# yangao07/abPOA

Measured on NVIDIA H100. Metric: GCUPS (DP cells/s), global/convex 10 kbp, higher is better.
Workload: dtype int16 (packed int16x2 DPX arithmetic; int32 kernel only as overflow fallback)

## Files before the change

### abpoa_b200/csrc/poa_chain.cu

```cuda
#include <cuda_runtime.h>
#include <algorithm>
#include <atomic>
#include <chrono>
#include <mutex>
#include <thread>
#include <vector>
#include <stddef.h>
#include <stdio.h>
#include <stdlib.h>
#include <string.h>
#include <unistd.h>
#include "abpoa_gpu.h"
#include "poa_internal.h"
#include "poa_engine.h"
#include "poa_device.cuh"
#include "poa_chain.cuh"
#include "poa_chain_host.h"

#define CK(call) do { cudaError_t e_ = (call); if (e_ != cudaSuccess) \
    poa_die("libabpoa_b200/chain", "%s failed at %s:%d: %s", #call, __FILE__, __LINE__, cudaGetErrorString(e_)); } while (0)

extern "C" cudaError_t poa_launch_chain_dp_worker(int gap_mode, const int *gaps, PoaChainSlot *slots, PoaChainSync *sync, int n_groups,
                                                  const PoaChainParams *cp, int strand, int ps, const PoaParamsDev *prm, int ring_rows, int ring_cells,
                                                  cudaStream_t st);
extern "C" cudaError_t poa_launch_chain_align_p16(int gap_mode, const int *gaps, const PoaChainSlot *slots, const int32_t *idx, int n_jobs, int round,
                                                  const PoaChainParams *cp, int strand, int ps, const PoaParamsDev *prm, int ring_rows, int ring_cells,
                                                  cudaStream_t st);
extern "C" void poa_pick_ring(int gap_mode, int bits, int band_cells, size_t smem_budget, int *ring_rows, int *ring_cells);

static_assert(offsetof(PoaChainSync, q_tail) == 128 && offsetof(PoaChainSync, total) == 256 && offsetof(PoaChainSync, abort) == 384,
              "every polled / bumped word of PoaChainSync sits in its own 128-byte line");
static_assert(POA_GFA_HDR_WORDS == POA_GFA_HDR, "the device's GFA record header is the one poa_gfa_from_record reads");

template <bool PS>
__global__ void __launch_bounds__(POA_CHAIN_T) poa_chain_seed_kernel(PoaChainSlot *slots, const PoaChainParams *cp, int n) {
    if ((int)blockIdx.x >= n) return;
    chain_seed<PS>(&slots[blockIdx.x], cp);
}

template <bool PS>
__global__ void __launch_bounds__(POA_CHAIN_T) poa_chain_fuse_kernel(PoaChainSlot *slots, const int32_t *idx, const PoaChainParams *cp, int n, int round) {
    if ((int)blockIdx.x >= n) return;
    chain_fuse<PS>(&slots[idx[blockIdx.x]], cp, round);
}

__device__ __forceinline__ int sync_ld(const int32_t *p) { int v; asm volatile("ld.relaxed.gpu.global.s32 %0, [%1];" : "=r"(v) : "l"(p) : "memory"); return v; }
__device__ __forceinline__ void sync_st(int32_t *p, int v) { asm volatile("st.relaxed.gpu.global.s32 [%0], %1;" :: "l"(p), "r"(v) : "memory"); }
__device__ __forceinline__ unsigned long long sync_now_ns() { unsigned long long t; asm volatile("mov.u64 %0, %%globaltimer;" : "=l"(t)); return t; }

template <bool PS>
__global__ void __launch_bounds__(POA_CHAIN_T) poa_chain_fuse_worker_kernel(PoaChainSlot *slots, PoaChainSync *sync, const PoaChainParams *cp) {
    __shared__ int task_s;
    for (;;) {
        if (threadIdx.x < 32) {
            unsigned ticket = 0;
            if (threadIdx.x == 0) ticket = atomicAdd(&sync->q_head, 1u);
            ticket = __shfl_sync(0xffffffffu, ticket, 0);
            int g = -2; unsigned ns = 250, polls = 0;
            const unsigned long long t0 = sync_now_ns(), limit = sync->watchdog_ns;
            const int32_t *tasks = sync->tasks;
            for (;;) {
                if ((polls++ & 31u) == 0) {
                    const int tot = __shfl_sync(0xffffffffu, sync_ld(&sync->total), 0), ab = __shfl_sync(0xffffffffu, sync_ld(&sync->abort), 0);
                    if ((long long)ticket >= (long long)tot || ab) { g = -2; break; }
                    const unsigned late = __shfl_sync(0xffffffffu, (unsigned)(polls > 1 && sync_now_ns() - t0 > limit), 0);
                    if (late) { if (threadIdx.x == 0) sync_st(&sync->abort, 1); g = -2; break; }
                }
                g = __shfl_sync(0xffffffffu, sync_ld(&tasks[ticket]), 0);
                if (g >= 0) break;
                __nanosleep(ns); if (ns < 4000) ns <<= 1;
            }
            if (threadIdx.x == 0) task_s = g;
        }
        __syncthreads();
        const int g = task_s;
        __syncthreads();
        if (g < 0) return;
        __threadfence();
        PoaChainSlot *s = &slots[g];
        const unsigned long long t0 = sync_now_ns();
        chain_fuse<PS>(s, cp, 0);
        __syncthreads();
        __threadfence();
        __syncthreads();
        if (threadIdx.x == 0) { s->fuse_ns += sync_now_ns() - t0; __threadfence(); sync_st(&s->turn, 0); }
    }
}

__global__ void __launch_bounds__(POA_CHAIN_T) poa_chain_export_kernel(PoaChainSlot *slots, const PoaChainParams *cp, int n,
                                                                       int32_t *ex, const int64_t *ex_off, const int32_t *ex_cap) {
    if ((int)blockIdx.x >= n) return;
    PoaChainSlot *s = &slots[blockIdx.x];
    int32_t *o = ex + ex_off[blockIdx.x];
    const int K = cp->K, A = cp->A, nn = s->n_nodes;
    if (s->failed) { if (threadIdx.x == 0) o[0] = -1; return; }
    int32_t *ci = s->scr[0], *ca = s->scr[1];
    POA_PAR_FOR(v, nn) { ci[v] = s->in_cnt[v]; ca[v] = s->aln_cnt[v]; }
    __syncthreads();
    const int n_in = cta_excl_scan(ci, nn);
    __syncthreads();
    const int n_aln = cta_excl_scan(ca, nn);
    __syncthreads();
    int32_t *co = s->scr[2];
    POA_PAR_FOR(v, nn) co[v] = s->out_cnt[v];
    __syncthreads();
    const int n_out = cta_excl_scan(co, nn);
    __syncthreads();
    const int64_t words = 4 + 5ll * nn + 4ll * n_in + n_aln;
    if (words > ex_cap[blockIdx.x] || n_out != n_in) { if (threadIdx.x == 0) o[0] = -1; return; }
    int32_t *base = o + 4, *n_read = base + nn, *in_cnt = n_read + nn, *out_cnt = in_cnt + nn, *aln_cnt = out_cnt + nn;
    int32_t *in_id = aln_cnt + nn, *in_w = in_id + n_in, *out_id = in_w + n_in, *out_w = out_id + n_in, *aln = out_w + n_in;
    if (threadIdx.x == 0) { o[0] = nn; o[1] = n_in; o[2] = n_aln; o[3] = s->fused; }
    POA_PAR_FOR(v, nn) {
        base[v] = s->base[v]; n_read[v] = s->n_read[v]; in_cnt[v] = s->in_cnt[v]; out_cnt[v] = s->out_cnt[v]; aln_cnt[v] = s->aln_cnt[v];
        for (int e = 0; e < s->in_cnt[v]; ++e) { in_id[ci[v] + e] = s->in_id[(size_t)v * K + e]; in_w[ci[v] + e] = s->in_w[(size_t)v * K + e]; }
        for (int e = 0; e < s->out_cnt[v]; ++e) { out_id[co[v] + e] = s->out_id[(size_t)v * K + e]; out_w[co[v] + e] = s->out_w[(size_t)v * K + e]; }
        for (int a = 0; a < s->aln_cnt[v]; ++a) aln[ca[v] + a] = s->aln_id[(size_t)v * A + a];
    }
}

__global__ void __launch_bounds__(POA_CHAIN_T) poa_chain_consensus_kernel(PoaChainSlot *slots, const PoaChainParams *cp, int n,
                                                                          int32_t *out, unsigned long long *cursor, unsigned long long out_words, int64_t *rec_off) {
    if ((int)blockIdx.x >= n) return;
    PoaChainSlot *s = &slots[blockIdx.x];
    int32_t *tmp = s->scr[2];
    chain_cons_path(s, cp, tmp, s->n_cap);
    if (threadIdx.x != 0) return;
    const int len = tmp[0];
    if (len < 0) { rec_off[blockIdx.x] = -1; return; }
    const unsigned long long at = atomicAdd(cursor, (unsigned long long)(len + 1));
    if (at + (unsigned long long)(len + 1) > out_words) { rec_off[blockIdx.x] = -1; return; }
    for (int k = 0; k <= len; ++k) out[at + k] = tmp[k];
    rec_off[blockIdx.x] = (int64_t)at;
}

__global__ void __launch_bounds__(POA_CHAIN_T) poa_chain_msa_kernel(PoaChainSlot *slots, const PoaChainParams *cp, int n, int with_cons, int run_cons,
                                                                    int32_t *out, unsigned long long *cursor, unsigned long long rec_base,
                                                                    unsigned long long out_words, int64_t *rec_off) {
    if ((int)blockIdx.x >= n) return;
    __shared__ long long at_s;
    __shared__ int len_s;
    PoaChainSlot *s = &slots[blockIdx.x];
    if (run_cons && !s->failed && s->n_nodes >= 3) chain_cons_path(s, cp, s->scr[2], s->n_cap);
    if (threadIdx.x == 0) {
        const int msa_len = chain_msa_rank(s, cp);
        long long at = -1;
        if (msa_len > 0) {
            const unsigned long long words = 2 + ((unsigned long long)(s->n_reads + with_cons) * (unsigned long long)msa_len + 3) / 4;
            const unsigned long long a = rec_base + atomicAdd(cursor, words);
            if (a + words <= out_words) at = (long long)a;
        }
        at_s = at; len_s = msa_len;
        rec_off[blockIdx.x] = at;
        if (at >= 0) { out[at] = msa_len; out[at + 1] = s->n_reads + with_cons; }
    }
    __syncthreads();
    if (at_s < 0) return;
    chain_msa_rows(s, cp, len_s, with_cons, reinterpret_cast<uint8_t *>(out + at_s + 2));
}

__global__ void __launch_bounds__(POA_CHAIN_T) poa_chain_gfa_kernel(PoaChainSlot *slots, const PoaChainParams *cp, int n, int with_cons, int run_cons,
                                                                    int32_t *out, unsigned long long *cursor, unsigned long long rec_base,
                                                                    unsigned long long out_words, int64_t *rec_off) {
    if ((int)blockIdx.x >= n) return;
    __shared__ long long at_s;
    __shared__ int32_t hdr_s[POA_GFA_HDR_WORDS];
    PoaChainSlot *s = &slots[blockIdx.x];
    if (run_cons && !s->failed && s->n_nodes >= 3) chain_cons_path(s, cp, s->scr[2], s->n_cap);
    if (threadIdx.x == 0) {
        const long long words = chain_gfa_size(s, cp, with_cons, hdr_s);
        long long at = -1;
        if (words > 0) {
            const unsigned long long a = (rec_base + atomicAdd(cursor, (unsigned long long)words + 1) + 1) & ~1ull;
            if (a + (unsigned long long)words <= out_words) at = (long long)a;
        }
        at_s = at;
        rec_off[blockIdx.x] = at;
    }
    __syncthreads();
    if (at_s < 0) return;
    chain_gfa_record(s, cp, hdr_s, out + at_s);
}

__global__ void poa_chain_path_score_kernel(const int32_t *edge_w, const int32_t *node_w, int n, int32_t *out) {
    for (int i = (int)(blockIdx.x * blockDim.x + threadIdx.x); i < n; i += (int)(gridDim.x * blockDim.x)) out[i] = chain_path_score(edge_w[i], node_w[i]);
}

static inline size_t al256(size_t x) { return (x + 255) & ~(size_t)255; }

extern "C" int poa_debug_path_scores(const int32_t *edge_w, const int32_t *node_w, int n, int32_t *out) {
    if (n <= 0) return 0;
    int32_t *d = NULL;
    const size_t b = (size_t)n * 4;
    CK(cudaMalloc((void **)&d, 3 * b));
    CK(cudaMemcpy(d, edge_w, b, cudaMemcpyHostToDevice));
    CK(cudaMemcpy(d + n, node_w, b, cudaMemcpyHostToDevice));
    poa_chain_path_score_kernel<<<(n + 255) / 256 < 4096 ? (n + 255) / 256 : 4096, 256>>>(d, d + n, n, d + 2 * (size_t)n);
    CK(cudaGetLastError());
    CK(cudaMemcpy(out, d + 2 * (size_t)n, b, cudaMemcpyDeviceToHost));
    CK(cudaFree(d));
    return n;
}

int poa_chain_eligible(const abpoa_para_t *abpt) {
    const char *off = getenv("ABPOA_GPU_NO_CHAIN");
    if (off && *off == '1') return 0;
    { const char *np = getenv("ABPOA_GPU_NO_P16"); if (np && *np == '1') return 0; }
    if (abpt->align_mode != ABPOA_GLOBAL_MODE || abpt->wb < 0) return 0;
    if (abpt->gap_mode == ABPOA_LINEAR_GAP) return 0;
    const int mf = abpt->cons_algrm == ABPOA_MF && abpt->use_read_ids && !abpt->sub_aln;
    if (abpt->cons_algrm != ABPOA_HB && !mf) return 0;
    if ((abpt->use_read_ids && !abpt->out_msa && !abpt->out_gfa && !mf) || abpt->max_n_cons > 1) return 0;
    if (abpt->zdrop > 0 || abpt->rev_cigar || !abpt->ret_cigar) return 0;
    if (abpt->put_gap_on_right || abpt->put_gap_at_end) return 0;
    if (abpt->m > POA_MAX_M) return 0;
    if (!(abpt->disable_seeding && abpt->progressive_poa == 0)) return 0;
    return 1;
}

namespace {

const int ROUNDS_EXTRA = 2;
int rounds_extra(bool strand, int n_reads) { return ROUNDS_EXTRA + (strand ? n_reads - 1 : 0); }
const double STRAND_SLAB_X = 5.0;

struct GroupPlan {
    int g;
    int n_reads, qmax; int64_t bases;
    int n_cap;
    size_t reads_bytes;
    size_t static_bytes;
    double pool_units_est;
    double rec_bytes;
};

struct Cohort {
    std::vector<int> members;
    cudaStream_t st = NULL;
    cudaEvent_t ev_end = NULL;
    std::vector<cudaEvent_t> marks;
};

double now_ms() { return std::chrono::duration<double, std::milli>(std::chrono::steady_clock::now().time_since_epoch()).count(); }

struct PinnedSlot { void *p = NULL; size_t cap = 0; bool busy = false; };
std::mutex g_pin_mu; PinnedSlot g_pin[4];
void *pinned_get(int which, size_t bytes) {
    std::lock_guard<std::mutex> lk(g_pin_mu);
    PinnedSlot &ps = g_pin[which];
    if (ps.busy) { void *q = NULL; CK(cudaHostAlloc(&q, bytes ? bytes : 1, cudaHostAllocPortable)); return q; }
    if (bytes > ps.cap) {
        if (ps.p) CK(cudaFreeHost(ps.p));
        ps.cap = bytes + bytes / 4 + 4096;
        CK(cudaHostAlloc(&ps.p, ps.cap, cudaHostAllocPortable));
    }
    ps.busy = true;
    return ps.p;
}
void pinned_put(int which, void *q) {
    std::lock_guard<std::mutex> lk(g_pin_mu);
    if (q == g_pin[which].p) g_pin[which].busy = false; else CK(cudaFreeHost(q));
}

bool launches_serialised() {
    static const bool serialised = [] {
        { const char *lb = getenv("CUDA_LAUNCH_BLOCKING"); if (lb && *lb == '1') return true; }
        for (char **v = environ; v && *v; ++v)
            if (!strncmp(*v, "CUDA_INJECTION64_PATH=", 22) || !strncmp(*v, "NV_NSIGHT_INJECTION", 19) || !strncmp(*v, "NV_COMPUTE_PROFILER", 19) ||
                !strncmp(*v, "NV_SANITIZER_INJECTION", 22) || !strncmp(*v, "NV_TPS_LAUNCH_", 14)) return true;
        if (FILE *mp = fopen("/proc/self/maps", "r")) {
            char line[512]; bool hit = false;
            while (!hit && fgets(line, sizeof line, mp))
                hit = strstr(line, "InjectionTarget") || strstr(line, "cuda-injection") || strstr(line, "libsanitizer-collection") || strstr(line, "TreeLauncherTarget");
            fclose(mp);
            if (hit) return true;
        }
        return false;
    }();
    return serialised;
}

struct ChainCall {
    int dev; poa_arena *arena; abpoa_para_t *abpt; int n_workers;
    const abpoa_gpu_group_t *groups; abpoa_gpu_group_result_t *results; PoaChainStats *stats; struct PoaEmit *emit;
    bool record, verbose;
    int m, K, A;
    int P;
    bool free_run;
    int cohorts;
    bool want_msa; int with_cons;
    bool mf;
    bool want_gfa;
    int W;
    bool export_graph;
    bool strand;
    bool qv;
    bool ps;
    int sm_count;
};

ChainCall chain_call(int dev, poa_arena *arena, abpoa_para_t *abpt, int n_workers, const abpoa_gpu_group_t *groups,
                     abpoa_gpu_group_result_t *results, const std::vector<int> &todo, int flags, PoaChainStats *stats, struct PoaEmit *emit) {
    ChainCall c;
    c.dev = dev; c.arena = arena; c.abpt = abpt; c.n_workers = n_workers; c.groups = groups; c.results = results; c.stats = stats; c.emit = emit;
    c.record = (flags & ABPOA_GPU_RECORD_READS) != 0;
    c.verbose = getenv("ABPOA_GPU_PROFILE") != NULL;
    c.m = abpt->m;
    { const char *e = getenv("ABPOA_GPU_CHAIN_K"); c.K = e && *e ? atoi(e) : (c.m > 5 ? 24 : 12); }
    c.A = c.m - 1 > 1 ? c.m - 1 : 1;
    c.P = abpt->gap_mode == ABPOA_LINEAR_GAP ? 1 : (abpt->gap_mode == ABPOA_AFFINE_GAP ? 2 : 3);
    { const char *e = getenv("ABPOA_GPU_CHAIN_COHORTS"); c.cohorts = !e ? 0 : std::max(1, std::min(16, *e ? atoi(e) : 4)); }
    const bool serialised = launches_serialised();
    { const char *e = getenv("ABPOA_GPU_CHAIN_ROUNDS"); c.free_run = e && *e ? *e != '1' : !serialised; }
    { const char *e = getenv("ABPOA_GPU_CHAIN_EXPORT_GRAPH"); c.export_graph = e && *e == '1'; }
    c.want_msa = abpt->out_msa && !abpt->out_gfa;
    c.want_gfa = abpt->out_gfa && emit != NULL;
    c.with_cons = abpt->out_cons ? 1 : 0;
    c.mf = abpt->cons_algrm == ABPOA_MF;
    c.strand = abpt->amb_strand != 0;
    c.ps = abpt->inc_path_score != 0;
    c.qv = false;
    if (abpt->use_qv)
        for (int g : todo)
            for (int i = 0; groups[g].qual_weights && i < groups[g].n_seq && !c.qv; ++i) c.qv = groups[g].qual_weights[i] != NULL;
    c.W = 0;
    if (c.want_msa || c.want_gfa) for (int g : todo) c.W = std::max(c.W, (groups[g].n_seq + 63) / 64);
    c.sm_count = 132;
    if (cudaDeviceGetAttribute(&c.sm_count, cudaDevAttrMultiProcessorCount, dev) != cudaSuccess || c.sm_count < 1) c.sm_count = 132;
    return c;
}

std::vector<GroupPlan> plan_groups(const ChainCall &c, const std::vector<int> &todo, std::vector<int> &fallback) {
    std::vector<GroupPlan> plans;
    for (int g : todo) {
        const abpoa_gpu_group_t &in = c.groups[g];
        GroupPlan p; p.g = g; p.n_reads = in.n_seq; p.qmax = 0; p.bases = 0;
        bool ok = in.n_seq >= 2;
        for (int i = 0; i < in.n_seq; ++i) {
            const int l = in.seq_lens[i];
            if (l < 1) ok = false;
            if (l > p.qmax) p.qmax = l;
            p.bases += l;
            if (ok && !poa_p16_ok(c.abpt, l, 3 * l)) ok = false;
            const int *qw = c.qv && in.qual_weights ? in.qual_weights[i] : NULL;
            for (int j = 0; ok && qw && j < l; ++j) ok = qw[j] >= 0 && qw[j] <= 255;
        }
        if (c.ps && (int64_t)in.n_seq * (c.qv ? 255 : 1) > POA_PS_MAX_NODE_W) ok = false;
        if (!ok || p.qmax > (1 << 24)) { fallback.push_back(g); continue; }
        const int64_t grow = std::min<int64_t>((int64_t)((double)p.qmax * (1.0 + 0.10 * (p.n_reads - 1))) + 256,
                                               (int64_t)((double)p.qmax * (1.0 + 0.04 * (p.n_reads - 1))) + 4096);
        p.n_cap = (int)std::min<int64_t>(2 + p.bases, grow);
        PoaChainSlot probe;
        size_t own = 0; p.reads_bytes = 0;
        chain_slot_layout(&probe, p.n_cap, p.qmax, p.n_reads, c.K, c.A, c.m, c.W, c.record, [&](size_t b) { own += al256(b); return (uint8_t *)NULL; }, c.strand, c.ps);
        chain_slot_reads(&probe, p.n_reads, p.bases, [&](size_t b) { p.reads_bytes += al256(b); return (uint8_t *)NULL; }, c.qv);
        p.static_bytes = own + p.reads_bytes;
        const size_t nc = (size_t)p.n_cap;
        p.rec_bytes = c.want_msa ? (double)(nc + 1) * 4 + 8 + (double)(p.n_reads + c.with_cons) * (double)nc + 1024 : 0.0;
        if (c.want_gfa)
            p.rec_bytes = (double)(nc + 1) * 4 + 4.0 * (POA_GFA_HDR_WORDS + 4 + 4.0 * (double)nc + (double)(p.bases + p.n_reads))
                        + 8.0 * (double)nc * (double)((p.n_reads + 63) / 64) + 1024;
        const int wmax = poa_band_halfwidth(c.abpt, p.qmax);
        const double growth = c.free_run ? 0.032 : 0.045;
        const int band_slack = c.free_run ? 0 : 32;
        const double rows_final = std::min<double>(2.0 + (double)p.bases, (double)p.qmax * (1.0 + growth * (p.n_reads - 1)) + 64);
        p.pool_units_est = rows_final * (double)((2 * wmax + 1 + band_slack + 7) / 8 + 2) * c.P;
        if (c.strand) p.pool_units_est *= STRAND_SLAB_X;
        plans.push_back(p);
    }
    return plans;
}

std::vector<std::pair<size_t, size_t>> split_waves(const std::vector<GroupPlan> &plans, size_t arena_cap, std::vector<int> &fallback) {
    const double pool_margin = 1.15;
    auto fit_from = [&](size_t from, size_t limit, size_t *need_static_out, double *need_pool_out) {
        size_t end = from, need_static = 0; double need_pool = 0;
        while (end < plans.size() && end - from < limit) {
            const size_t s2 = need_static + plans[end].static_bytes + sizeof(PoaChainSlot) + 4096;
            const double p2 = need_pool + std::max(plans[end].pool_units_est * 16.0 * pool_margin, plans[end].rec_bytes);
            if (end > from && (double)s2 + p2 + (64 << 20) > (double)arena_cap) break;
            need_static = s2; need_pool = p2; ++end;
        }
        if (need_static_out) *need_static_out = need_static;
        if (need_pool_out) *need_pool_out = need_pool;
        return end;
    };
    size_t n_waves = 0;
    for (size_t q = 0; q < plans.size(); ++n_waves) q = fit_from(q, plans.size(), NULL, NULL);
    const size_t per_wave = (plans.size() + n_waves - 1) / std::max<size_t>(n_waves, 1);
    std::vector<std::pair<size_t, size_t>> waves;
    for (size_t pos = 0; pos < plans.size();) {
        size_t need_static = 0; double need_pool = 0;
        const size_t end = fit_from(pos, per_wave, &need_static, &need_pool);
        if ((double)need_static + need_pool * 0.5 + (64 << 20) > (double)arena_cap) {
            fallback.push_back(plans[pos].g); ++pos; continue;
        }
        waves.push_back({pos, end});
        pos = end;
    }
    return waves;
}

struct Wave {
    const ChainCall &c;
    const GroupPlan *plans;
    const int nw;
    std::vector<int> &fallback;

    uint8_t *d_base = NULL; size_t total = 0, doff = 0;
    PoaChainSlot *d_slots = NULL; PoaChainParams *d_cp = NULL; PoaParamsDev *d_prm = NULL;
    unsigned long long *d_cursors = NULL;
    PoaChainSync *d_sync = NULL; int32_t *d_tasks = NULL; int64_t n_tasks = 0;
    uint8_t *d_reads = NULL; size_t reads_bytes = 0;
    int32_t *d_idx = NULL; size_t idx_n = 0;
    int64_t *d_exoff = NULL, *d_msaoff = NULL, *d_gfaoff = NULL; int32_t *d_excap = NULL;
    uint8_t *d_pool = NULL; size_t pool_bytes = 0; int32_t *d_ex = NULL;
    std::vector<PoaChainSlot> hs, fin;
    uint8_t *h_reads = NULL; int32_t *h_cons = NULL, *h_ex = NULL;
    std::vector<int64_t> h_exoff; std::vector<int32_t> h_excap; int64_t ex_words = 0;
    int band_cells = 64;
    std::vector<Cohort> coh;
    cudaStream_t s0 = NULL, st_dp = NULL;
    cudaEvent_t ev_up = NULL, ev_t0 = NULL, ev_t1 = NULL;
    int ring_rows = 2, ring_cells = 64; int gaps[4];
    bool cons_kernel = false; unsigned long long rec_base = 0, cons_words = 0;
    std::vector<int64_t> recoff, msaoff, gfaoff, words, hoff2; int64_t tot_words = 0;
    std::vector<std::vector<int32_t>> rs, rn; std::vector<std::vector<uint64_t>> rh;
    std::vector<std::vector<uint8_t>> rc;
    int n_failed = 0;
    int64_t launches = 0; uint64_t h2d = 0, d2h = 0; float dev_ms = 0.f;
    double t_wave0 = 0, t_staged = 0, t_uploaded = 0, t_enqueued = 0, t_dev_done = 0, t_copied = 0;

    Wave(const ChainCall &c_, const GroupPlan *plans_, int nw_, std::vector<int> &fallback_) : c(c_), plans(plans_), nw(nw_), fallback(fallback_) {}
    Wave(const Wave &) = delete;
    Wave &operator=(const Wave &) = delete;
    ~Wave() {
        if (d_base) poa_arena_return(c.arena, d_base, total);
        if (h_reads) pinned_put(0, h_reads);
        if (h_cons) pinned_put(2, h_cons);
        if (h_ex) pinned_put(3, h_ex);
        for (Cohort &k : coh) {
            for (cudaEvent_t ev : k.marks) cudaEventDestroy(ev);
            if (k.ev_end) cudaEventDestroy(k.ev_end);
            if (k.st) cudaStreamDestroy(k.st);
        }
        if (st_dp) cudaStreamDestroy(st_dp);
        for (cudaEvent_t ev : { ev_up, ev_t0, ev_t1 }) if (ev) cudaEventDestroy(ev);
    }

    uint8_t *dtake(size_t b) { uint8_t *q = d_base + doff; doff += al256(b); return q; }

    void run() {
        if (!carve_and_stage()) {
            for (int t = 0; t < nw; ++t) fallback.push_back(plans[t].g);
            return;
        }
        if (c.free_run) run_free_running(); else run_rounds();
        collect();
        install();
        account();
    }

    bool carve_and_stage() {
        t_wave0 = now_ms();
        total = poa_arena_capacity(c.arena);
        d_base = poa_arena_borrow(c.arena, total);
        d_slots = (PoaChainSlot *)dtake((size_t)nw * sizeof(PoaChainSlot));
        d_cp = (PoaChainParams *)dtake(sizeof(PoaChainParams));
        d_prm = (PoaParamsDev *)dtake(sizeof(PoaParamsDev));
        d_cursors = (unsigned long long *)dtake((size_t)32 * sizeof(unsigned long long));
        d_sync = (PoaChainSync *)dtake(sizeof(PoaChainSync));
        for (int t = 0; t < nw; ++t) n_tasks += plans[t].n_reads - 1;
        d_tasks = (int32_t *)dtake((size_t)std::max<int64_t>(n_tasks, 1) * 4);
        for (int t = 0; t < nw; ++t) reads_bytes += plans[t].reads_bytes;
        h_reads = (uint8_t *)pinned_get(0, reads_bytes + 256);
        d_reads = dtake(reads_bytes);
        size_t roff = 0;
        auto rtake = [&](size_t b) { uint8_t *q = d_reads + roff; roff += al256(b); return q; };
        auto gtake = [&](size_t b) { return dtake(b); };
        hs.resize((size_t)nw);
        for (int t = 0; t < nw; ++t) {
            const GroupPlan &p = plans[t];
            const abpoa_gpu_group_t &in = c.groups[p.g];
            PoaChainSlot &s = hs[t]; memset(&s, 0, sizeof s);
            chain_slot_layout(&s, p.n_cap, p.qmax, p.n_reads, c.K, c.A, c.m, c.W, c.record, gtake, c.strand, c.ps);
            chain_slot_reads(&s, p.n_reads, p.bases, rtake, c.qv);
            int32_t *hoff = (int32_t *)(h_reads + ((const uint8_t *)s.read_off - d_reads)), *hw = (int32_t *)(h_reads + ((const uint8_t *)s.read_w - d_reads));
            int acc = 0;
            for (int i = 0; i < p.n_reads; ++i) {
                hoff[i] = acc; acc += in.seq_lens[i];
                hw[i] = poa_band_halfwidth(c.abpt, in.seq_lens[i]);
                const int bc = (2 * hw[i] + 1 + 104 + 7) / 8 * 8;
                if (bc > band_cells) band_cells = bc;
            }
            hoff[p.n_reads] = acc;
        }
        {
            std::atomic<int> nx(0);
            auto copy_reads = [&]() {
                for (int t; (t = nx.fetch_add(1)) < nw;) {
                    const abpoa_gpu_group_t &in = c.groups[plans[t].g];
                    uint8_t *q = h_reads + (hs[t].reads - d_reads);
                    for (int i = 0; i < in.n_seq; ++i) { memcpy(q, in.seqs[i], (size_t)in.seq_lens[i]); q += in.seq_lens[i]; }
                    if (!c.qv) continue;
                    uint8_t *w = h_reads + (hs[t].read_qw - d_reads);
                    for (int i = 0; i < in.n_seq; ++i) {
                        const int *qw = in.qual_weights ? in.qual_weights[i] : NULL;
                        if (qw) for (int j = 0; j < in.seq_lens[i]; ++j) w[j] = (uint8_t)qw[j];
                        else memset(w, 1, (size_t)in.seq_lens[i]);
                        w += in.seq_lens[i];
                    }
                }
            };
            const int nth = reads_bytes < (8u << 20) ? 1 : std::max(1, std::min(c.n_workers, 16));
            std::vector<std::thread> th;
            for (int w = 1; w < nth; ++w) th.emplace_back(copy_reads);
            copy_reads();
            for (auto &x : th) x.join();
        }
        t_staged = now_ms();
        idx_n = (size_t)n_tasks;
        for (int t = 0; t < nw; ++t) idx_n += (size_t)rounds_extra(c.strand, plans[t].n_reads);
        d_idx = (int32_t *)dtake(std::max<size_t>(idx_n, 1) * 4);
        h_exoff.resize((size_t)nw); h_excap.resize((size_t)nw);
        for (int t = 0; t < nw; ++t) {
            const GroupPlan &p = plans[t];
            const int64_t cap = 4 + 5ll * p.n_cap + 4ll * 3 * p.n_cap + (int64_t)p.n_cap * 2;
            h_exoff[t] = ex_words; h_excap[t] = (int32_t)std::min<int64_t>(cap, INT32_MAX); ex_words += (cap + 63) & ~63ll;
        }
        d_exoff = (int64_t *)dtake((size_t)nw * 8); d_excap = (int32_t *)dtake((size_t)nw * 4);
        d_msaoff = c.want_msa ? (int64_t *)dtake((size_t)nw * 8) : NULL;
        d_gfaoff = c.want_gfa ? (int64_t *)dtake((size_t)nw * 8) : NULL;
        doff = al256(doff);
        if (doff > total) poa_die("libabpoa_b200/chain", "wave layout (%zu bytes) exceeds the arena (%zu bytes)", doff, total);
        if (doff + (size_t)ex_words * 4 + (32 << 20) > total) return false;
        d_pool = d_base + doff; pool_bytes = total - doff;
        d_ex = (int32_t *)d_pool;
        return true;
    }

    void upload_and_seed(const std::vector<int32_t> &idx) {
        for (Cohort &k : coh) { CK(cudaStreamCreateWithFlags(&k.st, cudaStreamNonBlocking)); CK(cudaEventCreate(&k.ev_end)); }
        s0 = coh[0].st;
        CK(cudaEventCreateWithFlags(&ev_up, cudaEventDisableTiming)); CK(cudaEventCreate(&ev_t0)); CK(cudaEventCreate(&ev_t1));
        const abpoa_para_t *abpt = c.abpt;
        PoaChainParams hcp; memset(&hcp, 0, sizeof hcp);
        hcp.K = c.K; hcp.A = c.A; hcp.m = c.m; hcp.max_mat = abpt->max_mat; hcp.min_mis = abpt->min_mis; hcp.o1 = abpt->gap_open1; hcp.e1 = abpt->gap_ext1;
        hcp.oe1 = abpt->gap_open1 + abpt->gap_ext1; hcp.oe2 = abpt->gap_open2 + abpt->gap_ext2; hcp.record = c.record ? 1 : 0; hcp.P = c.P; hcp.W = c.W;
        hcp.cons_algrm = c.mf ? 1 : 0; hcp.amb_strand = c.strand ? 1 : 0;
        PoaParamsDev hprm; poa_fill_params(&hprm, c.abpt, 15);
        CK(cudaMemcpyAsync(d_reads, h_reads, reads_bytes, cudaMemcpyHostToDevice, s0));
        CK(cudaMemcpyAsync(d_slots, hs.data(), (size_t)nw * sizeof(PoaChainSlot), cudaMemcpyHostToDevice, s0));
        CK(cudaMemcpyAsync(d_cp, &hcp, sizeof hcp, cudaMemcpyHostToDevice, s0));
        CK(cudaMemcpyAsync(d_prm, &hprm, sizeof hprm, cudaMemcpyHostToDevice, s0));
        if (!idx.empty()) CK(cudaMemcpyAsync(d_idx, idx.data(), idx.size() * 4, cudaMemcpyHostToDevice, s0));
        CK(cudaMemcpyAsync(d_exoff, h_exoff.data(), (size_t)nw * 8, cudaMemcpyHostToDevice, s0));
        CK(cudaMemcpyAsync(d_excap, h_excap.data(), (size_t)nw * 4, cudaMemcpyHostToDevice, s0));
        CK(cudaMemsetAsync(d_cursors, 0, (size_t)32 * sizeof(unsigned long long), s0));
        h2d = reads_bytes + (uint64_t)nw * sizeof(PoaChainSlot) + sizeof hcp + sizeof hprm + idx.size() * 4 + (uint64_t)nw * 12;
        CK(cudaEventRecord(ev_t0, s0));
        if (c.ps) poa_chain_seed_kernel<true><<<nw, POA_CHAIN_T, 0, s0>>>(d_slots, d_cp, nw);
        else poa_chain_seed_kernel<false><<<nw, POA_CHAIN_T, 0, s0>>>(d_slots, d_cp, nw);
        CK(cudaGetLastError());
        CK(cudaEventRecord(ev_up, s0));
        static const size_t smem_budget = [] { const char *e = getenv("ABPOA_GPU_SMEM_KB"); return (size_t)(e && *e ? atoi(e) : 28) * 1024; }();
        poa_pick_ring(abpt->gap_mode, 16, band_cells, smem_budget, &ring_rows, &ring_cells);
        launches = 1;
        gaps[0] = abpt->gap_ext1; gaps[1] = abpt->gap_open1 + abpt->gap_ext1; gaps[2] = abpt->gap_ext2; gaps[3] = abpt->gap_open2 + abpt->gap_ext2;
        t_uploaded = now_ms();
        for (size_t k = 1; k < coh.size(); ++k) CK(cudaStreamWaitEvent(coh[k].st, ev_up, 0));
    }

    void run_free_running() {
        coh.resize(1);
        double est_tot = 0;
        for (int t = 0; t < nw; ++t) est_tot += plans[t].pool_units_est;
        static const double slab_x = [] { const char *e = getenv("ABPOA_GPU_CHAIN_SLAB_X"); return e && *e ? atof(e) : 0.0; }();
        size_t o = 0;
        for (int t = 0; t < nw; ++t) {
            size_t share = (size_t)((double)pool_bytes * plans[t].pool_units_est / est_tot) & ~(size_t)255;
            if (slab_x > 0) share = std::min(share, (size_t)(plans[t].pool_units_est * 16.0 * slab_x) & ~(size_t)255);
            hs[t].pool_base = d_pool + o; hs[t].pool_units = share / 16; hs[t].pool_cursor = NULL;
            o += share;
        }
        upload_and_seed({});
        static const double watchdog_s = [] { const char *e = getenv("ABPOA_GPU_CHAIN_WATCHDOG_S"); return e && *e ? atof(e) : 30.0; }();
        static const int fuse_per_sm = [] { const char *e = getenv("ABPOA_GPU_CHAIN_FUSE_PER_SM"); return e && *e ? std::max(1, atoi(e)) : 1; }();
        PoaChainSync hsync; memset(&hsync, 0, sizeof hsync);
        hsync.total = (int32_t)n_tasks; hsync.watchdog_ns = (unsigned long long)(watchdog_s * 1e9); hsync.tasks = d_tasks;
        CK(cudaMemcpyAsync(d_sync, &hsync, sizeof hsync, cudaMemcpyHostToDevice, s0));
        CK(cudaMemsetAsync(d_tasks, 0xff, (size_t)std::max<int64_t>(n_tasks, 1) * 4, s0));
        CK(cudaStreamCreateWithFlags(&st_dp, cudaStreamNonBlocking));
        cudaEvent_t ev_sync; CK(cudaEventCreateWithFlags(&ev_sync, cudaEventDisableTiming));
        CK(cudaEventRecord(ev_sync, s0));
        static const int fuse_cap = [] { const char *e = getenv("ABPOA_GPU_CHAIN_FUSE_WORKERS"); return e && *e ? std::max(1, atoi(e)) : (1 << 30); }();
        const int n_fuse = std::max(1, std::min(std::min(nw, c.sm_count * fuse_per_sm), fuse_cap));
        CK(cudaFuncSetAttribute(c.ps ? poa_chain_fuse_worker_kernel<true> : poa_chain_fuse_worker_kernel<false>, cudaFuncAttributePreferredSharedMemoryCarveout,
                                cudaSharedmemCarveoutMaxShared));
        static const bool dp_first = [] { const char *e = getenv("ABPOA_GPU_CHAIN_DP_FIRST"); return e && *e == '1'; }();
        CK(cudaStreamWaitEvent(st_dp, ev_sync, 0));
        if (dp_first) CK(poa_launch_chain_dp_worker(c.abpt->gap_mode, gaps, d_slots, d_sync, nw, d_cp, c.strand, c.ps, d_prm, ring_rows, ring_cells, st_dp));
        if (c.ps) poa_chain_fuse_worker_kernel<true><<<n_fuse, POA_CHAIN_T, 0, s0>>>(d_slots, d_sync, d_cp);
        else poa_chain_fuse_worker_kernel<false><<<n_fuse, POA_CHAIN_T, 0, s0>>>(d_slots, d_sync, d_cp);
        CK(cudaGetLastError());
        if (!dp_first) CK(poa_launch_chain_dp_worker(c.abpt->gap_mode, gaps, d_slots, d_sync, nw, d_cp, c.strand, c.ps, d_prm, ring_rows, ring_cells, st_dp));
        cudaEvent_t ev_dp; CK(cudaEventCreateWithFlags(&ev_dp, cudaEventDisableTiming));
        CK(cudaEventRecord(ev_dp, st_dp));
        CK(cudaStreamWaitEvent(s0, ev_dp, 0));
        CK(cudaEventDestroy(ev_sync)); CK(cudaEventDestroy(ev_dp));
        launches += 2;
    }

    void run_rounds() {
        const int n_coh = c.cohorts ? c.cohorts : std::max(1, std::min(16, (nw + c.sm_count - 1) / c.sm_count));
        coh.resize((size_t)std::min(n_coh, nw));
        for (int t = 0; t < nw; ++t) coh[(size_t)t % coh.size()].members.push_back(t);
        std::vector<double> est(coh.size(), 0.0); double est_tot = 0;
        for (size_t k = 0; k < coh.size(); ++k) { for (int t : coh[k].members) est[k] += plans[t].pool_units_est; est_tot += est[k]; }
        size_t o = 0;
        for (size_t k = 0; k < coh.size(); ++k) {
            const size_t share = k + 1 == coh.size() ? pool_bytes - o : (size_t)((double)pool_bytes * est[k] / est_tot) & ~(size_t)255;
            for (int t : coh[k].members) { hs[t].pool_base = d_pool + o; hs[t].pool_units = share / 16; hs[t].pool_cursor = d_cursors + 2 * k; }
            o += share;
        }
        std::vector<int32_t> h_idx; std::vector<std::vector<std::pair<size_t, int>>> round_of(coh.size());
        int n_rounds = 0;
        for (int t = 0; t < nw; ++t) n_rounds = std::max(n_rounds, plans[t].n_reads - 1 + rounds_extra(c.strand, plans[t].n_reads));
        for (size_t k = 0; k < coh.size(); ++k)
            for (int r = 1; r <= n_rounds; ++r) {
                const size_t at = h_idx.size(); int cnt = 0;
                for (int t : coh[k].members) if (plans[t].n_reads + rounds_extra(c.strand, plans[t].n_reads) > r) { h_idx.push_back(t); ++cnt; }
                round_of[k].push_back({at, cnt});
            }
        if (h_idx.size() != idx_n) poa_die("libabpoa_b200/chain", "round index lists (%zu entries) do not fill their region (%zu)", h_idx.size(), idx_n);
        upload_and_seed(h_idx);
        for (int r = 1; r <= n_rounds; ++r)
            for (size_t k = 0; k < coh.size(); ++k) {
                cudaStream_t st = coh[k].st;
                const std::pair<size_t, int> &ro = round_of[k][(size_t)r - 1];
                if (ro.second == 0) continue;
                cudaEvent_t e0, e1, e2; CK(cudaEventCreate(&e0)); CK(cudaEventCreate(&e1)); CK(cudaEventCreate(&e2));
                coh[k].marks.push_back(e0); coh[k].marks.push_back(e1); coh[k].marks.push_back(e2);
                CK(cudaEventRecord(e0, st));
                CK(poa_launch_chain_align_p16(c.abpt->gap_mode, gaps, d_slots, d_idx + ro.first, ro.second, r, d_cp, c.strand, c.ps, d_prm, ring_rows, ring_cells, st));
                CK(cudaEventRecord(e1, st));
                if (c.ps) poa_chain_fuse_kernel<true><<<ro.second, POA_CHAIN_T, 0, st>>>(d_slots, d_idx + ro.first, d_cp, ro.second, r);
                else poa_chain_fuse_kernel<false><<<ro.second, POA_CHAIN_T, 0, st>>>(d_slots, d_idx + ro.first, d_cp, ro.second, r);
                CK(cudaGetLastError());
                CK(cudaEventRecord(e2, st));
                launches += 2;
            }
    }

    void collect() {
        for (size_t k = 0; k < coh.size(); ++k) CK(cudaEventRecord(coh[k].ev_end, coh[k].st));
        t_enqueued = now_ms();
        for (size_t k = 1; k < coh.size(); ++k) CK(cudaStreamWaitEvent(s0, coh[k].ev_end, 0));
        CK(cudaEventRecord(ev_t1, s0));
        const bool export_graph = c.export_graph, want_msa = c.want_msa, want_gfa = c.want_gfa;
        unsigned long long *d_ccur = d_cursors;
        int64_t *d_recoff = d_exoff;
        if (c.abpt->out_gfa) cons_kernel = !export_graph && want_gfa && c.with_cons;
        else cons_kernel = !export_graph && (!want_msa || c.with_cons);
        const bool any_rec = cons_kernel || want_msa || want_gfa;
        rec_base = export_graph ? (unsigned long long)ex_words : 0;
        if (export_graph) poa_chain_export_kernel<<<nw, POA_CHAIN_T, 0, s0>>>(d_slots, d_cp, nw, d_ex, d_exoff, d_excap);
        if (any_rec) CK(cudaMemsetAsync(d_ccur, 0, sizeof(unsigned long long), s0));
        if (cons_kernel) poa_chain_consensus_kernel<<<nw, c.mf ? POA_CHAIN_T : 32, 0, s0>>>(d_slots, d_cp, nw, d_ex, d_ccur, (unsigned long long)(pool_bytes / 4), d_recoff);
        CK(cudaGetLastError());
        launches += (export_graph || cons_kernel) ? 1 : 0;
        if (want_msa) {
            poa_chain_msa_kernel<<<nw, POA_CHAIN_T, 0, s0>>>(d_slots, d_cp, nw, c.with_cons, export_graph && c.with_cons, d_ex, d_ccur, rec_base,
                                                            (unsigned long long)(pool_bytes / 4), d_msaoff);
            CK(cudaGetLastError());
            ++launches;
        }
        if (want_gfa) {
            poa_chain_gfa_kernel<<<nw, POA_CHAIN_T, 0, s0>>>(d_slots, d_cp, nw, c.with_cons, export_graph && c.with_cons, d_ex, d_ccur, rec_base,
                                                            (unsigned long long)(pool_bytes / 4), d_gfaoff);
            CK(cudaGetLastError());
            ++launches;
        }
        fin.resize((size_t)nw);
        PoaChainSlot *h_fin = (PoaChainSlot *)pinned_get(1, (size_t)nw * sizeof(PoaChainSlot));
        CK(cudaMemcpyAsync(h_fin, d_slots, (size_t)nw * sizeof(PoaChainSlot), cudaMemcpyDeviceToHost, s0));
        CK(cudaStreamSynchronize(s0));
        CK(cudaEventElapsedTime(&dev_ms, ev_t0, ev_t1));
        memcpy(fin.data(), h_fin, (size_t)nw * sizeof(PoaChainSlot));
        pinned_put(1, h_fin);
        if (c.free_run) {
            PoaChainSync hs2; CK(cudaMemcpy(&hs2, d_sync, sizeof hs2, cudaMemcpyDeviceToHost));
            if (hs2.abort) fprintf(stderr, "[libabpoa_b200/chain] watchdog: the alignment and the fuse kernel did not make progress together within ABPOA_GPU_CHAIN_WATCHDOG_S; "
                                           "unfinished groups go to the launch engine (ABPOA_GPU_CHAIN_ROUNDS=1 selects the round schedule)\n");
        }
        t_dev_done = now_ms();
        recoff.assign((size_t)nw, -1); msaoff.assign((size_t)nw, -1); gfaoff.assign((size_t)nw, -1);
        if (any_rec) {
            int64_t *h_ro = NULL; CK(cudaHostAlloc((void **)&h_ro, (size_t)nw * 24 + 8, cudaHostAllocDefault));
            if (cons_kernel) CK(cudaMemcpyAsync(h_ro, d_recoff, (size_t)nw * 8, cudaMemcpyDeviceToHost, s0));
            if (want_msa) CK(cudaMemcpyAsync(h_ro + nw, d_msaoff, (size_t)nw * 8, cudaMemcpyDeviceToHost, s0));
            if (want_gfa) CK(cudaMemcpyAsync(h_ro + 2 * nw, d_gfaoff, (size_t)nw * 8, cudaMemcpyDeviceToHost, s0));
            CK(cudaMemcpyAsync(h_ro + 3 * nw, d_ccur, 8, cudaMemcpyDeviceToHost, s0));
            CK(cudaStreamSynchronize(s0));
            if (cons_kernel) memcpy(recoff.data(), h_ro, (size_t)nw * 8);
            if (want_msa) memcpy(msaoff.data(), h_ro + nw, (size_t)nw * 8);
            if (want_gfa) memcpy(gfaoff.data(), h_ro + 2 * nw, (size_t)nw * 8);
            cons_words = (unsigned long long)h_ro[3 * nw];
            CK(cudaFreeHost(h_ro));
            if (rec_base + cons_words > pool_bytes / 4) cons_words = pool_bytes / 4 - rec_base;
            h_cons = (int32_t *)pinned_get(2, (size_t)std::max<unsigned long long>(cons_words, 1) * 4);
            if (cons_words) CK(cudaMemcpyAsync(h_cons, d_ex + rec_base, (size_t)cons_words * 4, cudaMemcpyDeviceToHost, s0));
        }
        std::vector<int32_t> hdr4((size_t)nw * 4);
        if (export_graph) {
            int32_t *h_hdr = NULL; CK(cudaHostAlloc((void **)&h_hdr, (size_t)nw * 16, cudaHostAllocDefault));
            for (int t = 0; t < nw; ++t) CK(cudaMemcpyAsync(h_hdr + 4 * t, d_ex + h_exoff[t], 16, cudaMemcpyDeviceToHost, s0));
            CK(cudaStreamSynchronize(s0));
            memcpy(hdr4.data(), h_hdr, (size_t)nw * 16);
            CK(cudaFreeHost(h_hdr));
        }
        words.assign((size_t)nw, 0); hoff2.assign((size_t)nw, 0);
        for (int t = 0; t < nw; ++t) {
            const bool rec_ok = (!cons_kernel || recoff[t] >= 0) && (!want_msa || msaoff[t] >= 0) && (!want_gfa || gfaoff[t] >= 0);
            if (!export_graph) { words[t] = (!fin[t].failed && rec_ok) ? 1 : 0; continue; }
            if (fin[t].failed || hdr4[4 * t] < 2 || !rec_ok) continue;
            words[t] = 4 + 5ll * hdr4[4 * t] + 4ll * hdr4[4 * t + 1] + hdr4[4 * t + 2];
            hoff2[t] = tot_words; tot_words += words[t];
        }
        h_ex = (int32_t *)pinned_get(3, (size_t)std::max<int64_t>(tot_words, 1) * 4);
        if (export_graph) for (int t = 0; t < nw; ++t) if (words[t]) CK(cudaMemcpyAsync(h_ex + hoff2[t], d_ex + h_exoff[t], (size_t)words[t] * 4, cudaMemcpyDeviceToHost, s0));
        rs.resize((size_t)nw); rn.resize((size_t)nw); rh.resize((size_t)nw);
        if (c.record) for (int t = 0; t < nw; ++t) {
            const int nr = plans[t].n_reads;
            rs[t].resize(nr); rn[t].resize(nr); rh[t].resize(nr);
            CK(cudaMemcpyAsync(rs[t].data(), fin[t].rec_score, (size_t)nr * 4, cudaMemcpyDeviceToHost, s0));
            CK(cudaMemcpyAsync(rn[t].data(), fin[t].rec_nops, (size_t)nr * 4, cudaMemcpyDeviceToHost, s0));
            CK(cudaMemcpyAsync(rh[t].data(), fin[t].rec_hash, (size_t)nr * 8, cudaMemcpyDeviceToHost, s0));
        }
        rc.resize((size_t)nw);
        uint64_t rc_bytes = 0;
        if (c.strand) for (int t = 0; t < nw; ++t) {
            rc[t].resize((size_t)plans[t].n_reads);
            CK(cudaMemcpyAsync(rc[t].data(), fin[t].read_rc, (size_t)plans[t].n_reads, cudaMemcpyDeviceToHost, s0));
            rc_bytes += (uint64_t)plans[t].n_reads;
        }
        CK(cudaStreamSynchronize(s0));
        d2h = (uint64_t)tot_words * 4 + (uint64_t)cons_words * 4 + (uint64_t)nw * (sizeof(PoaChainSlot) + 16) + rc_bytes;
        poa_arena_return(c.arena, d_base, total); d_base = NULL;
        t_copied = now_ms();
    }

    void install() {
        std::atomic<int> next(0), failed(0);
        std::vector<int> failed_groups; std::mutex fmu;
        const int nth = std::max(1, std::min(c.n_workers, nw));
        std::vector<std::thread> th;
        for (int w = 0; w < nth; ++w)
            th.emplace_back([&]() {
                abpoa_para_t *abpt = c.abpt;
                abpoa_t *ab = abpoa_init();
                for (;;) {
                    const int t = next.fetch_add(1);
                    if (t >= nw) break;
                    const GroupPlan &p = plans[t];
                    if (fin[t].failed || !words[t] || fin[t].fused != p.n_reads) {
                        if (c.verbose) fprintf(stderr, "[chain] group %d left the device chain after %d reads (flags 0x%x)\n", p.g, fin[t].fused, fin[t].failed);
                        std::lock_guard<std::mutex> lk(fmu); failed_groups.push_back(p.g); failed += 1; continue;
                    }
                    abpoa_gpu_group_result_t *o = &c.results[p.g];
                    memset(o, 0, sizeof *o);
                    abpoa_reset(ab, abpt, p.qmax);
                    abpoa_seq_t *abs = ab->abs;
                    abs->n_seq = p.n_reads; poa_seq_reserve(abs);
                    int n_rc_dp = 0;
                    for (int i = 0; i < p.n_reads; ++i) {
                        abs->is_rc[i] = c.strand ? rc[t][i] & 1 : 0; abs->name[i].l = 0;
                        if (c.strand) n_rc_dp += rc[t][i] >> 1 & 1;
                    }
                    if (c.export_graph) poa_graph_import(ab, abpt, h_ex + hoff2[t]);
                    else if (cons_kernel) {
                        const int32_t *rec = h_cons + recoff[t];
                        const int len = rec[0];
                        std::vector<uint8_t> cb((size_t)(len > 0 ? len : 1)); std::vector<int> cc((size_t)(len > 0 ? len : 1));
                        for (int j = 0; j < len; ++j) { cb[j] = (uint8_t)(rec[1 + j] & 0xff); cc[j] = rec[1 + j] >> 8; }
                        poa_cons_install(ab, p.n_reads, len, cb.data(), cc.data());
                    }
                    if (c.want_msa) {
                        const int32_t *rec = h_cons + (msaoff[t] - (int64_t)rec_base);
                        poa_msa_install(ab, p.n_reads, rec[1], rec[0], reinterpret_cast<const uint8_t *>(rec + 2));
                    }
                    if (c.want_gfa) poa_gfa_install(ab, h_cons + (gfaoff[t] - (int64_t)rec_base));
                    poa_finish_group_result(ab, abpt, o, c.emit, p.g);
                    if (c.want_gfa) poa_gfa_install(ab, NULL);
                    o->dp_cells = fin[t].cells; o->n_aligned = p.n_reads - 1 + n_rc_dp;
                    if (c.record) {
                        const int nr = p.n_reads;
                        o->read_best_score = (int32_t *)poa_xcalloc((size_t)nr, sizeof(int32_t));
                        o->read_n_cigar = (int32_t *)poa_xcalloc((size_t)nr, sizeof(int32_t));
                        o->read_cigar_hash = (uint64_t *)poa_xcalloc((size_t)nr, sizeof(uint64_t));
                        o->read_cigar_hash[0] = 1469598103934665603ull;
                        for (int i = 1; i < nr; ++i) { o->read_best_score[i] = rs[t][i]; o->read_n_cigar[i] = rn[t][i]; o->read_cigar_hash[i] = rh[t][i]; }
                    }
                }
                abpoa_free(ab);
            });
        for (auto &x : th) x.join();
        for (int g : failed_groups) fallback.push_back(g);
        n_failed = failed.load();
    }

    void account() {
        int64_t cells = 0, alns = 0, fwd_clk = 0, bt_clk = 0;
        for (int t = 0; t < nw; ++t) if (!fin[t].failed && words[t] && fin[t].fused == plans[t].n_reads) { cells += fin[t].cells; alns += plans[t].n_reads - 1; fwd_clk += fin[t].fwd_clk; bt_clk += fin[t].bt_clk; }
        double dp_ms = 0, fuse_ms = 0, wait_ms = 0; int64_t n_marks = 0;
        if (c.free_run) {
            int khz = 0; if (cudaDeviceGetAttribute(&khz, cudaDevAttrClockRate, c.dev) != cudaSuccess || khz <= 0) khz = 1965000;
            for (int t = 0; t < nw; ++t) {
                dp_ms += (double)(fin[t].fwd_clk + fin[t].bt_clk) / (double)khz; fuse_ms += (double)fin[t].fuse_ns * 1e-6; wait_ms += (double)fin[t].wait_ns * 1e-6;
                n_marks += fin[t].fused > 0 ? fin[t].fused - 1 : 0;
            }
        } else {
            for (Cohort &k : coh)
                for (size_t j = 0; j + 2 < k.marks.size(); j += 3) {
                    float a = 0.f, b = 0.f;
                    CK(cudaEventElapsedTime(&a, k.marks[j], k.marks[j + 1])); CK(cudaEventElapsedTime(&b, k.marks[j + 1], k.marks[j + 2]));
                    dp_ms += a; fuse_ms += b; ++n_marks;
                }
        }
        if (PoaChainStats *stats = c.stats) {
            stats->device_ms += dev_ms; stats->cells += cells; stats->alignments += alns; stats->launches += launches;
            stats->h2d_bytes += h2d; stats->d2h_bytes += d2h; stats->groups_done += nw - n_failed; stats->groups_failed += n_failed;
            stats->fwd_clk += fwd_clk; stats->bt_clk += bt_clk;
            stats->dp_ms += dp_ms; stats->fuse_ms += fuse_ms; stats->dp_launches += n_marks; stats->fuse_launches += n_marks;
            stats->wait_ms += wait_ms; stats->free_running = c.free_run ? 1 : 0;
        }
        if (!c.verbose) return;
#ifdef POA_KPROF
        {
            double pf[6] = {0, 0, 0, 0, 0, 0}; double na = 0;
            for (int t = 0; t < nw; ++t) { for (int z = 0; z < 6; ++z) pf[z] += (double)fin[t].prof[z]; na += fin[t].fused > 0 ? fin[t].fused - 1 : 0; }
            double bd[5] = {0, 0, 0, 0, 0};
            for (int t = 0; t < nw; ++t) for (int z = 0; z < 5; ++z) bd[z] += (double)fin[t].btdiag[z];
            if (na > 0) fprintf(stderr, "[chain, backtrace per alignment] %.0f steps in %.0f speculative rounds, %.0f general steps costing %.0f k-cycles, "
                                        "%.1f rows with their F planes recomputed\n", bd[0] / na, bd[1] / na, bd[2] / na, bd[3] / na, bd[4] / na);
            if (na > 0) fprintf(stderr, "[chain, k-cycles/alignment] -DPOA_KPROF phases: setup %.0f pred %.0f compute %.0f store %.0f rowmax %.0f tail+prefetch %.0f\n",
                                pf[0] / na / 1e3, pf[1] / na / 1e3, pf[2] / na / 1e3, pf[3] / na / 1e3, pf[4] / na / 1e3, pf[5] / na / 1e3);
        }
#endif
        if (c.free_run)
            fprintf(stderr, "[chain] free-running: per group on average %.1f ms inside alignments + %.1f ms inside fuse (waited %.1f ms for fuse workers incl. the fuse itself), %lld alignments\n",
                    dp_ms / nw, fuse_ms / nw, wait_ms / nw, (long long)n_marks);
        else
            fprintf(stderr, "[chain] DP kernels %.1f ms + fuse kernels %.1f ms summed over %zu concurrent cohort streams (%lld rounds)\n", dp_ms, fuse_ms, coh.size(), (long long)n_marks);
        fprintf(stderr, "[chain] wave of %d groups (%zu cohorts, K=%d): stage %.0f + upload-enqueue %.0f + launch-enqueue %.0f ms, stage+launch+device %.0f ms (device %.1f ms), export copy %.0f ms, import+consensus %.0f ms; "
                        "static %.2f GB, pool %.2f GB, export %.1f MB; %d groups handed to the launch engine\n",
                nw, coh.size(), c.K, t_staged - t_wave0, t_uploaded - t_staged, t_enqueued - t_uploaded, t_dev_done - t_wave0, dev_ms, t_copied - t_dev_done, now_ms() - t_copied,
                (double)doff / 1e9, (double)pool_bytes / 1e9, (double)tot_words * 4 / 1e6, n_failed);
    }
};

}

int poa_chain_run(int dev, poa_arena *arena, abpoa_para_t *abpt, int n_workers, const abpoa_gpu_group_t *groups,
                  abpoa_gpu_group_result_t *results, const std::vector<int> &todo, int flags, std::vector<int> &fallback, PoaChainStats *stats,
                  struct PoaEmit *emit) {
    CK(cudaSetDevice(dev));
    const ChainCall c = chain_call(dev, arena, abpt, n_workers, groups, results, todo, flags, stats, emit);
    const std::vector<GroupPlan> plans = plan_groups(c, todo, fallback);
    if (plans.empty()) return 0;
    for (const std::pair<size_t, size_t> &w : split_waves(plans, poa_arena_capacity(arena), fallback))
        Wave(c, plans.data() + w.first, (int)(w.second - w.first), fallback).run();
    return 0;
}
```

### abpoa_b200/csrc/poa_chain.cuh

```cuda
#ifndef POA_CHAIN_CUH
#define POA_CHAIN_CUH

#include <math.h>
#include <stdint.h>
#include "poa_device.cuh"

#ifdef POA_CHAIN_EMUL
#define POA_DEV static inline
#define POA_PAR_FOR(i, n) for (int i = 0; i < (n); ++i)
#define POA_CTA_SYNC() do { } while (0)
#define POA_TID0 1
#define POA_SHARED static
#define POA_ATOMIC_OR(p, v) (*(p) |= (v))
#define POA_CTZ64(x) __builtin_ctzll(x)
#define POA_CHAIN_T 256
#else
#define POA_DEV __device__ __forceinline__
#define POA_PAR_FOR(i, n) for (int i = (int)threadIdx.x; i < (n); i += (int)blockDim.x)
#define POA_CTA_SYNC() __syncthreads()
#define POA_TID0 (threadIdx.x == 0)
#define POA_SHARED __shared__
#define POA_ATOMIC_OR(p, v) atomicOr((p), (v))
#define POA_CTZ64(x) (__ffsll((long long)(x)) - 1)
#define POA_CHAIN_T 256
#endif

#define POA_CF_NODE_CAP   0x01
#define POA_CF_EDGE_CAP   0x02
#define POA_CF_ALN_CAP    0x04
#define POA_CF_ORDER      0x08
#define POA_CF_BLOB_CAP   0x10
#define POA_CF_DP_STATUS  0x20
#define POA_CF_CIGAR      0x40
#define POA_CF_POOL       0x80

#define POA_ST_SKIP       9

typedef struct PoaChainParams {
    int32_t K, A;
    int32_t m, max_mat, min_mis, o1, e1, oe1, oe2;
    int32_t record;
    int32_t P;
    int32_t W;
    int32_t cons_algrm;
    int32_t amb_strand;
} PoaChainParams;

typedef struct PoaChainSlot {
    int32_t n_nodes, n_cap, pred_cap, blob_cap;
    int32_t failed;
    int32_t n_reads, fused;
    int32_t retry;
    int32_t cur;
    int64_t cells;
    int64_t fwd_clk, bt_clk;
    uint8_t *base;
    int32_t *in_cnt, *out_cnt, *aln_cnt, *n_read;
    int32_t *in_id, *in_w, *out_id, *out_w;
    int32_t *aln_id;
    int32_t *order[2];
    int32_t *node_row;
    int32_t *rem_row;
    int32_t *scr[6];
    const uint8_t *reads; const int32_t *read_off;
    const int32_t *read_w;
    PoaJobDesc jd;
    uint8_t *pool_base; unsigned long long *pool_cursor; uint64_t pool_units;
    int32_t turn;
    int32_t rsv0;
    unsigned long long wait_ns, fuse_ns;
    int64_t prof[6];
    int64_t btdiag[5];
    int32_t *rec_score, *rec_nops; uint64_t *rec_hash;
    uint64_t *read_set;
    uint8_t *read_rc;
    uint64_t *rc_cigar;
    PoaResultDev *rc_result;
    const uint8_t *read_qw;
} PoaChainSlot;

template <class Take>
static inline void chain_slot_layout(PoaChainSlot *s, int n_cap, int qmax, int n_reads, int K, int A, int m, int W, bool record, Take take,
                                     bool strand = false, bool ps = false) {
    const size_t nc = (size_t)n_cap, scr_n = nc > (size_t)qmax + 2 ? nc : (size_t)qmax + 2;
    s->n_cap = n_cap; s->pred_cap = (int32_t)(nc * 3); s->n_reads = n_reads;
    s->blob_cap = (int32_t)(256 + (nc + 1) * 8 + (size_t)s->pred_cap * 4 + 4 + (size_t)qmax + 64);
    if (ps) s->blob_cap += (int32_t)((size_t)s->pred_cap * 4 + 4 + 16);
    s->jd.cigar_cap = (int32_t)(qmax + n_cap + 8);
    s->base = (uint8_t *)take(nc);
    s->in_cnt = (int32_t *)take(nc * 4); s->out_cnt = (int32_t *)take(nc * 4); s->aln_cnt = (int32_t *)take(nc * 4); s->n_read = (int32_t *)take(nc * 4);
    s->in_id = (int32_t *)take(nc * K * 4); s->in_w = (int32_t *)take(nc * K * 4); s->out_id = (int32_t *)take(nc * K * 4); s->out_w = (int32_t *)take(nc * K * 4);
    s->aln_id = (int32_t *)take(nc * A * 4);
    s->order[0] = (int32_t *)take(nc * 4); s->order[1] = (int32_t *)take(nc * 4); s->node_row = (int32_t *)take(nc * 4); s->rem_row = (int32_t *)take(nc * 4);
    for (int k = 0; k < 6; ++k) s->scr[k] = (int32_t *)take(scr_n * 4);
    s->jd.blob = (uint8_t *)take((size_t)s->blob_cap);
    s->jd.rowinfo = (PoaRowInfo *)take(nc * sizeof(PoaRowInfo)); s->jd.rowoff = (PoaRowOff *)take(nc * sizeof(PoaRowOff));
    s->jd.cigar = (uint64_t *)take((size_t)s->jd.cigar_cap * 8);
    s->jd.qprof = (int16_t *)take((size_t)m * ((((size_t)qmax + 1 + 7) & ~(size_t)7) + 8) * 2);
    s->jd.result = (PoaResultDev *)take(sizeof(PoaResultDev));
    s->jd.btrec = (PoaBtRec *)take(nc * sizeof(PoaBtRec));
    if (record) { s->rec_score = (int32_t *)take((size_t)n_reads * 4); s->rec_nops = (int32_t *)take((size_t)n_reads * 4); s->rec_hash = (uint64_t *)take((size_t)n_reads * 8); }
    if (W > 0) s->read_set = (uint64_t *)take(nc * W * 8);
    if (strand) {
        s->read_rc = (uint8_t *)take((size_t)n_reads);
        s->rc_cigar = (uint64_t *)take((size_t)s->jd.cigar_cap * 8);
        s->rc_result = (PoaResultDev *)take(sizeof(PoaResultDev));
    }
}

template <class Take>
static inline void chain_slot_reads(PoaChainSlot *s, int n_reads, int64_t bases, Take take, bool qv = false) {
    s->reads = (const uint8_t *)take((size_t)bases);
    s->read_off = (const int32_t *)take(((size_t)n_reads + 1) * 4);
    s->read_w = (const int32_t *)take((size_t)n_reads * 4);
    if (qv) s->read_qw = (const uint8_t *)take((size_t)bases);
}

typedef struct PoaChainSync {
    unsigned int q_head; int32_t pad0[31];
    unsigned int q_tail; int32_t pad1[31];
    int32_t total; int32_t pad2[31];
    int32_t abort; int32_t pad3[31];
    unsigned long long watchdog_ns;
    int32_t *tasks;
} PoaChainSync;

#ifdef POA_CHAIN_EMUL
POA_DEV int cta_excl_scan(int32_t *a, int n) {
    int run = 0;
    for (int i = 0; i < n; ++i) { const int v = a[i]; a[i] = run; run += v; }
    return run;
}
POA_DEV void cta_incl_maxscan(int32_t *a, int n) {
    int run = INT32_MIN;
    for (int i = 0; i < n; ++i) { if (a[i] > run) run = a[i]; a[i] = run; }
}
#else
__device__ inline int cta_excl_scan(int32_t *a, int n) {
    __shared__ int warp_sum[32];
    __shared__ int carry_s;
    const int lane = threadIdx.x & 31, wid = threadIdx.x >> 5, nw = blockDim.x >> 5;
    if (threadIdx.x == 0) carry_s = 0;
    __syncthreads();
    for (int base = 0; base < n; base += blockDim.x) {
        const int i = base + threadIdx.x;
        const int v = i < n ? a[i] : 0;
        int x = v;
#pragma unroll
        for (int d = 1; d < 32; d <<= 1) { const int t = __shfl_up_sync(0xffffffffu, x, d); if (lane >= d) x += t; }
        if (lane == 31) warp_sum[wid] = x;
        __syncthreads();
        if (wid == 0) {
            int s = lane < nw ? warp_sum[lane] : 0;
#pragma unroll
            for (int d = 1; d < 32; d <<= 1) { const int t = __shfl_up_sync(0xffffffffu, s, d); if (lane >= d) s += t; }
            warp_sum[lane] = s;
        }
        __syncthreads();
        const int carry = carry_s;
        const int before = carry + (wid > 0 ? warp_sum[wid - 1] : 0) + x - v;
        if (i < n) a[i] = before;
        __syncthreads();
        if (threadIdx.x == 0) carry_s = carry + warp_sum[nw - 1];
        __syncthreads();
    }
    return carry_s;
}
__device__ inline void cta_incl_maxscan(int32_t *a, int n) {
    __shared__ int warp_max[32];
    __shared__ int carry_m;
    const int lane = threadIdx.x & 31, wid = threadIdx.x >> 5, nw = blockDim.x >> 5;
    if (threadIdx.x == 0) carry_m = INT32_MIN;
    __syncthreads();
    for (int base = 0; base < n; base += blockDim.x) {
        const int i = base + threadIdx.x;
        int x = i < n ? a[i] : INT32_MIN;
#pragma unroll
        for (int d = 1; d < 32; d <<= 1) { const int t = __shfl_up_sync(0xffffffffu, x, d); if (lane >= d) x = max(x, t); }
        if (lane == 31) warp_max[wid] = x;
        __syncthreads();
        if (wid == 0) {
            int s = lane < nw ? warp_max[lane] : INT32_MIN;
#pragma unroll
            for (int d = 1; d < 32; d <<= 1) { const int t = __shfl_up_sync(0xffffffffu, s, d); if (lane >= d) s = max(s, t); }
            warp_max[lane] = s;
        }
        __syncthreads();
        int r = max(carry_m, x);
        if (wid > 0) r = max(r, warp_max[wid - 1]);
        if (i < n) a[i] = r;
        __syncthreads();
        if (threadIdx.x == 0) carry_m = max(carry_m, warp_max[nw - 1]);
        __syncthreads();
    }
}
#endif

POA_DEV void chain_exchange_order(int32_t *ids, int32_t *ws, int n) {
    for (int j = 0; j + 1 < n; ++j)
        for (int k = j + 1; k < n; ++k)
            if (ws[j] < ws[k]) { int32_t t = ids[j]; ids[j] = ids[k]; ids[k] = t; t = ws[j]; ws[j] = ws[k]; ws[k] = t; }
}

POA_DEV int chain_group_last_row(const PoaChainSlot *s, int A, const int32_t *order, int old_n, int v) {
    int r = s->node_row[v];
    const int na = s->aln_cnt[v];
    if (na == 0) return r;
    const int32_t *al = s->aln_id + (size_t)v * A;
    for (; r + 1 < old_n; ++r) {
        const int u = order[r + 1];
        int member = 0;
        for (int a = 0; a < na; ++a) if (al[a] == u) { member = 1; break; }
        if (!member) break;
    }
    return r;
}

POA_DEV int chain_ref_pn(const PoaChainParams *cp, int qlen, int n_rows) {
    const int len = qlen > n_rows ? qlen : n_rows;
    const int a = qlen * cp->max_mat, b = len * cp->e1 + cp->o1;
    const int max_score = a > b ? a : b;
    return max_score <= 32767 - cp->min_mis - cp->oe1 - cp->oe2 ? 16 : 8;
}

POA_DEV size_t chain_al16(size_t x) { return (x + 15) & ~(size_t)15; }

POA_DEV bool chain_weak_hit(int best_score, int qlen, int node_n, int max_mat) {
    const int lim = qlen < node_n - 2 ? qlen : node_n - 2;
    return best_score < lim * max_mat * .3333;
}

#define POA_PS_MAX_NODE_W (1 << 20)
POA_DEV int chain_path_score(int edge_w, int node_w) {
    if (node_w == 0 || edge_w == 0) return 0;
    const int s = (int)round(log((double)edge_w / (double)node_w));
    return s > -20 ? s : -20;
}

POA_DEV uint8_t chain_comp(uint8_t b) { return b < 4 ? (uint8_t)(3 - b) : (uint8_t)4; }

typedef struct ChainRead { const uint8_t *q, *w; int len; bool rc; } ChainRead;

POA_DEV ChainRead chain_read(const PoaChainSlot *s, int r) {
    ChainRead rd;
    rd.q = s->reads + s->read_off[r]; rd.w = s->read_qw ? s->read_qw + s->read_off[r] : NULL;
    rd.len = s->read_off[r + 1] - s->read_off[r]; rd.rc = s->read_rc && (s->read_rc[r] & 1);
    return rd;
}

POA_DEV uint8_t chain_read_base(const ChainRead &rd, int qi) { return rd.rc ? chain_comp(rd.q[rd.len - 1 - qi]) : rd.q[qi]; }

POA_DEV int chain_read_weight(const ChainRead &rd, int qi) { return !rd.w ? 1 : rd.w[rd.rc ? rd.len - 1 - qi : qi]; }

POA_DEV void chain_set_remain(PoaChainSlot *s, int K, const int32_t *order, int n) {
    POA_SHARED int t_ptr[POA_CHAIN_T], t_val[POA_CHAIN_T], t_np[POA_CHAIN_T], t_nv[POA_CHAIN_T];
    int32_t *rem = s->rem_row;
    if (POA_TID0) rem[n - 1] = -1;
    POA_CTA_SYNC();
    for (int hi = n - 1; hi > 0; hi -= POA_CHAIN_T) {
        const int lo = hi - POA_CHAIN_T > 0 ? hi - POA_CHAIN_T : 0;
        const int cnt = hi - lo;
        POA_PAR_FOR(l, POA_CHAIN_T) {
            if (l < cnt) {
                const int v = order[lo + l];
                const int sr = s->node_row[s->out_id[(size_t)v * K]];
                if (sr >= hi) { t_ptr[l] = -1; t_val[l] = rem[sr] + 1; }
                else { t_ptr[l] = sr - lo; t_val[l] = 1; }
            } else { t_ptr[l] = -1; t_val[l] = 0; }
        }
        POA_CTA_SYNC();
        for (int step = 1; step < POA_CHAIN_T; step <<= 1) {
            POA_PAR_FOR(l, POA_CHAIN_T) {
                const int p = t_ptr[l];
                if (p >= 0) { t_nv[l] = t_val[l] + t_val[p]; t_np[l] = t_ptr[p]; } else { t_nv[l] = t_val[l]; t_np[l] = -1; }
            }
            POA_CTA_SYNC();
            POA_PAR_FOR(l, POA_CHAIN_T) { t_val[l] = t_nv[l]; t_ptr[l] = t_np[l]; }
            POA_CTA_SYNC();
        }
        POA_PAR_FOR(l, POA_CHAIN_T) { if (l < cnt) rem[lo + l] = t_val[l]; }
        POA_CTA_SYNC();
    }
}

template <bool PS = false>
POA_DEV void chain_flatten(PoaChainSlot *s, const PoaChainParams *cp, const int32_t *order, int n, int r, int pool_parity, int generous) {
    const int K = cp->K;
    int32_t *cnt = s->scr[0];
    POA_PAR_FOR(i, n) cnt[i] = i == 0 ? 0 : s->in_cnt[order[i]];
    POA_CTA_SYNC();
    const int n_pred = cta_excl_scan(cnt, n);
    POA_CTA_SYNC();
    const int qlen = s->read_off[r + 1] - s->read_off[r];
    uint8_t *blob = const_cast<uint8_t *>(s->jd.blob);
    PoaJobHeader *h = reinterpret_cast<PoaJobHeader *>(blob);
    size_t off = chain_al16(sizeof(PoaJobHeader));
    const size_t off_rowmeta = off; off += chain_al16(((size_t)n + 1) * 8);
    const size_t off_pred = off; off += chain_al16((size_t)n_pred * 4 + 4);
    const size_t off_ps = off; if (PS) off += chain_al16((size_t)n_pred * 4 + 4);
    const size_t off_qs = off; off += chain_al16((size_t)qlen + 1) + 16;
    if (off > (size_t)s->blob_cap || n_pred > s->pred_cap) {
        if (POA_TID0) { POA_ATOMIC_OR(&s->failed, POA_CF_BLOB_CAP); h->n_rows = 0; }
        POA_CTA_SYNC();
        return;
    }
    int32_t *rowmeta = reinterpret_cast<int32_t *>(blob + off_rowmeta), *pred = reinterpret_cast<int32_t *>(blob + off_pred);
    int32_t *pscore = reinterpret_cast<int32_t *>(blob + off_ps);
    uint8_t *qs = blob + off_qs;
    POA_PAR_FOR(i, n) {
        const int v = order[i];
        const int po = cnt[i];
        rowmeta[2 * i] = po;
        rowmeta[2 * i + 1] = (int32_t)((uint32_t)s->rem_row[i] << 8) | s->base[v];
        if (i > 0) {
            const int ni = s->in_cnt[v];
            const int32_t *iid = s->in_id + (size_t)v * K;
            for (int e = 0; e < ni; ++e) {
                const int pr = s->node_row[iid[e]];
                if (pr >= i) POA_ATOMIC_OR(&s->failed, POA_CF_ORDER);
                pred[po + e] = pr;
                if (PS) {
                    const int u = iid[e], no = s->out_cnt[u];
                    const int32_t *ow = s->out_w + (size_t)u * K;
                    int node_w = 0;
                    for (int o = 0; o < no; ++o) node_w += ow[o];
                    pscore[po + e] = chain_path_score(s->in_w[(size_t)v * K + e], node_w);
                }
            }
        }
    }
    const uint8_t *q = s->reads + s->read_off[r];
    const int qpad = (int)(off - off_qs);
    POA_PAR_FOR(j, qpad) qs[j] = (j >= 1 && j <= qlen) ? q[j - 1] : (uint8_t)0;
    if (POA_TID0) {
        rowmeta[2 * n] = n_pred; rowmeta[2 * n + 1] = 0;
        h->qlen = qlen; h->w = s->read_w[r]; h->node_n = n;
        h->off_rowmeta = (int32_t)off_rowmeta; h->off_pred = (int32_t)off_pred; h->off_predscore = PS ? (int32_t)off_ps : -1; h->off_live = -1;
        h->off_qs = (int32_t)off_qs; h->rsv[0] = h->rsv[1] = h->rsv[2] = h->rsv[3] = 0;
        h->blob_bytes = (int32_t)off; h->pn = chain_ref_pn(cp, qlen, n); h->pad[0] = h->pad[1] = 0;
#ifndef POA_CHAIN_EMUL
        if (s->pool_base) {
            const int w = s->read_w[r];
            const int drift = qlen > s->rem_row[0] ? qlen - s->rem_row[0] : s->rem_row[0] - qlen;
            unsigned long long per_row = (unsigned long long)((2 * w + 1 + drift + 64 + 7) / 8 + 2);
            const unsigned long long full = (unsigned long long)((qlen + 1 + 7) / 8 + 1);
            if (generous || per_row > full) per_row = full;
            const unsigned long long units = per_row * (unsigned long long)cp->P * (unsigned long long)n;
            if (!s->pool_cursor) {
                s->jd.planes = s->pool_base; s->jd.plane_cap_units = s->pool_units;
            } else {
                const unsigned long long at = atomicAdd(&s->pool_cursor[pool_parity & 1], units);
                if (at + units > s->pool_units) POA_ATOMIC_OR(&s->failed, POA_CF_POOL);
                else { s->jd.planes = s->pool_base + (size_t)at * (POA_GROUP * 2); s->jd.plane_cap_units = units; }
            }
        }
#endif
    }
    POA_CTA_SYNC();
    if (POA_TID0) h->n_rows = s->failed ? 0 : n;
    POA_CTA_SYNC();
}

template <bool PS = false>
POA_DEV void chain_seed(PoaChainSlot *s, const PoaChainParams *cp) {
    const int K = cp->K;
    ChainRead rd = chain_read(s, 0);
    rd.rc = false;
    const int len = rd.len;
    const uint8_t *q = rd.q;
    const int n = len + 2;
    if (n > s->n_cap || len < 1) {
        if (POA_TID0) { POA_ATOMIC_OR(&s->failed, POA_CF_NODE_CAP); reinterpret_cast<PoaJobHeader *>(const_cast<uint8_t *>(s->jd.blob))->n_rows = 0; }
        POA_CTA_SYNC();
        return;
    }
    int32_t *order = s->order[0];
    POA_PAR_FOR(v, n) {
        s->aln_cnt[v] = 0;
        if (v == 0) { s->base[v] = 0; s->in_cnt[v] = 0; s->out_cnt[v] = 1; s->out_id[0] = 2; s->out_w[0] = chain_read_weight(rd, 0); s->n_read[v] = 1; order[0] = 0; s->node_row[0] = 0; }
        else if (v == 1) {
            s->base[v] = 0; s->out_cnt[v] = 0; s->in_cnt[v] = 1; s->in_id[(size_t)K] = len + 1; s->in_w[(size_t)K] = chain_read_weight(rd, len - 1); s->n_read[v] = 0;
            order[n - 1] = 1; s->node_row[1] = n - 1;
        } else {
            const int i = v - 2;
            s->base[v] = q[i];
            s->in_cnt[v] = 1; s->in_id[(size_t)v * K] = i == 0 ? 0 : v - 1; s->in_w[(size_t)v * K] = chain_read_weight(rd, i);
            s->out_cnt[v] = 1; s->out_id[(size_t)v * K] = i == len - 1 ? 1 : v + 1; s->out_w[(size_t)v * K] = chain_read_weight(rd, i == len - 1 ? i : i + 1);
            s->n_read[v] = 1;
            order[i + 1] = v; s->node_row[v] = i + 1;
        }
    }
    if (cp->W > 0) {
        const int W = cp->W;
        POA_PAR_FOR(v, n) { uint64_t *rs = s->read_set + (size_t)v * W; for (int wd = 0; wd < W; ++wd) rs[wd] = (wd == 0 && v != 1) ? 1ull : 0ull; }
    }
    if (POA_TID0) { s->n_nodes = n; s->cur = 0; s->fused = 1; s->retry = 0; if (s->read_rc) s->read_rc[0] = 0; }
    POA_CTA_SYNC();
    chain_set_remain(s, K, order, n);
    if (s->n_reads > 1) chain_flatten<PS>(s, cp, order, n, 1, 1, 0);
}

#define CK_OLD  0
#define CK_NEWM 1
#define CK_NEWI 2

template <bool PS = false>
POA_DEV void chain_fuse(PoaChainSlot *s, const PoaChainParams *cp, int round) {
    const int K = cp->K, A = cp->A;
    const int r = s->fused;
    PoaJobHeader *hdr = reinterpret_cast<PoaJobHeader *>(const_cast<uint8_t *>(s->jd.blob));
    if (s->failed || r >= s->n_reads) return;
    const PoaResultDev *res = s->jd.result;
    if (res->status == POA_ST_SKIP) return;
    if (res->status == POA_ST_PLANE_OVF && !s->retry && s->pool_cursor) {
        POA_CTA_SYNC();
        if (POA_TID0) s->retry = 1;
        chain_flatten<PS>(s, cp, s->order[s->cur], s->n_nodes, r, round + 1, 1);
        return;
    }
    if (res->status != POA_ST_OK) {
        if (POA_TID0) { POA_ATOMIC_OR(&s->failed, POA_CF_DP_STATUS); hdr->n_rows = 0; }
        POA_CTA_SYNC();
        return;
    }
    const ChainRead rd = chain_read(s, r);
    const int qlen = rd.len;
    const uint64_t *ops = s->jd.cigar;
    const int n_ops = res->n_ops;
    const int old_n = s->n_nodes;
    const int32_t *order = s->order[s->cur];
    int32_t *order_new = s->order[s->cur ^ 1];
    int32_t *item_row = s->scr[0], *tgt = s->scr[1], *isnew = s->scr[2], *kind_anchor = s->scr[3], *defidx = s->scr[4], *new_anchor = s->scr[5];

    if (POA_TID0) {
        s->cells += res->cells; s->fwd_clk += res->fwd_clk; s->bt_clk += res->bt_clk;
#ifdef POA_KPROF
        for (int z = 0; z < 6; ++z) s->prof[z] += res->prof[z];
        for (int z = 0; z < 5; ++z) s->btdiag[z] += res->btdiag[z];
#endif
        if (cp->record) {
            s->rec_score[r] = res->best_score; s->rec_nops[r] = n_ops;
            uint64_t hsh = 1469598103934665603ull;
            for (int t = n_ops - 1; t >= 0; --t) {
                uint64_t w = ops[t];
                if ((w & 0xf) != 1) w = ((uint64_t)(uint32_t)order[w >> 34] << 34) | (w & 0x3ffffffffull);
                for (int b = 0; b < 8; ++b) { hsh ^= (w >> (8 * b)) & 0xff; hsh *= 1099511628211ull; }
            }
            s->rec_hash[r] = hsh;
        }
    }

    POA_PAR_FOR(qi, qlen + 1) { item_row[qi] = -2; }
    POA_CTA_SYNC();
    POA_PAR_FOR(t, n_ops) {
        const uint64_t w = ops[t];
        const int op = (int)(w & 0xf);
        if (op == 0) {
            const int qp = (int)((w >> 4) & 0x3fffffff), row = (int)(w >> 34);
            if (qp < qlen && row > 0 && row < old_n - 1) item_row[qp] = row; else POA_ATOMIC_OR(&s->failed, POA_CF_CIGAR);
        } else if (op == 1) {
            const int qp = (int)(w >> 34), len = (int)((w >> 4) & 0x3fffffff);
            if (qp < qlen && qp - len + 1 >= 0) { for (int k = 0; k < len; ++k) item_row[qp - k] = -1; } else POA_ATOMIC_OR(&s->failed, POA_CF_CIGAR);
        }
    }
    POA_CTA_SYNC();

    POA_PAR_FOR(qi, qlen) {
        const int row = item_row[qi];
        int kind = CK_NEWI, target = -1, anchor = -1;
        if (row == -2) POA_ATOMIC_OR(&s->failed, POA_CF_CIGAR);
        if (row >= 0) {
            const int v = order[row];
            const uint8_t b = chain_read_base(rd, qi);
            if (s->base[v] == b) { kind = CK_OLD; target = v; }
            else {
                const int na = s->aln_cnt[v]; const int32_t *al = s->aln_id + (size_t)v * A;
                for (int a = 0; a < na; ++a) if (s->base[al[a]] == b) { target = al[a]; break; }
                if (target >= 0) kind = CK_OLD;
                else { kind = CK_NEWM; anchor = chain_group_last_row(s, A, order, old_n, v); target = v; }
            }
        }
        tgt[qi] = target; isnew[qi] = kind != CK_OLD;
        kind_anchor[qi] = (kind << 28) | (anchor & 0x0fffffff);
    }
    POA_CTA_SYNC();
    if (s->failed) { if (POA_TID0) hdr->n_rows = 0; POA_CTA_SYNC(); return; }

    int32_t *newidx = defidx;
    POA_PAR_FOR(qi, qlen) newidx[qi] = isnew[qi];
    POA_CTA_SYNC();
    const int n_new = cta_excl_scan(newidx, qlen);
    POA_CTA_SYNC();
    const int n = old_n + n_new;
    if (n > s->n_cap) { if (POA_TID0) { POA_ATOMIC_OR(&s->failed, POA_CF_NODE_CAP); hdr->n_rows = 0; } POA_CTA_SYNC(); return; }

    POA_PAR_FOR(qi, qlen) {
        const int kind = kind_anchor[qi] >> 28;
        int anchor = -1;
        if (kind == CK_NEWM) anchor = kind_anchor[qi] & 0x0fffffff;
        else if (kind == CK_NEWI && !(qi > 0 && isnew[qi - 1])) anchor = chain_group_last_row(s, A, order, old_n, qi == 0 ? 0 : tgt[qi - 1]);
        new_anchor[qi] = anchor;
    }
    POA_CTA_SYNC();
    {
        int32_t *d = item_row;
        POA_PAR_FOR(qi, qlen) d[qi] = new_anchor[qi] >= 0 ? qi : -1;
        POA_CTA_SYNC();
        cta_incl_maxscan(d, qlen);
        POA_CTA_SYNC();
        POA_PAR_FOR(qi, qlen) {
            if (isnew[qi]) {
                const int a = d[qi] >= 0 ? new_anchor[d[qi]] : -1;
                if (a < 0) POA_ATOMIC_OR(&s->failed, POA_CF_ORDER);
                kind_anchor[qi] = (kind_anchor[qi] & (int32_t)0xf0000000) | (a & 0x0fffffff);
            }
        }
        POA_CTA_SYNC();
    }

    POA_PAR_FOR(qi, qlen) {
        if (isnew[qi]) {
            const int id = old_n + newidx[qi];
            const int col = tgt[qi];
            s->base[id] = chain_read_base(rd, qi); s->in_cnt[id] = 0; s->out_cnt[id] = 0; s->aln_cnt[id] = 0; s->n_read[id] = 0;
            if (cp->W > 0) for (int wd = 0; wd < cp->W; ++wd) s->read_set[(size_t)id * cp->W + wd] = 0;
            new_anchor[newidx[qi]] = kind_anchor[qi] & 0x0fffffff;
            item_row[qi] = col;
            tgt[qi] = id;
        }
    }
    POA_CTA_SYNC();

    POA_PAR_FOR(qi, qlen + 1) {
        const int from = qi == 0 ? 0 : tgt[qi - 1], to = qi < qlen ? tgt[qi] : 1;
        const int from_new = qi > 0 && isnew[qi - 1], to_new = qi < qlen && isnew[qi];
        const int w = chain_read_weight(rd, qi < qlen ? qi : qlen - 1);
        int32_t *iid = s->in_id + (size_t)to * K, *iw = s->in_w + (size_t)to * K;
        int32_t *oid = s->out_id + (size_t)from * K, *ow = s->out_w + (size_t)from * K;
        int nin = s->in_cnt[to], nout = s->out_cnt[from];
        int found = 0;
        if (!from_new && !to_new) {
            for (int i = 0; i < nin; ++i)
                if (iid[i] == from) { iw[i] += w; found = 1; if (i > 0 && iw[i - 1] < iw[i]) chain_exchange_order(iid, iw, nin); break; }
            if (found)
                for (int i = 0; i < nout; ++i)
                    if (oid[i] == to) { ow[i] += w; if (i > 0 && ow[i - 1] < ow[i]) chain_exchange_order(oid, ow, nout); break; }
        }
        if (!found) {
            if (nin >= K || nout >= K) POA_ATOMIC_OR(&s->failed, POA_CF_EDGE_CAP);
            else {
                iid[nin] = from; iw[nin] = w; s->in_cnt[to] = ++nin;
                if (nin > 1 && iw[nin - 2] < w) chain_exchange_order(iid, iw, nin);
                oid[nout] = to; ow[nout] = w; s->out_cnt[from] = ++nout;
                if (nout > 1 && ow[nout - 2] < w) chain_exchange_order(oid, ow, nout);
            }
        }
        s->n_read[from] += 1;
        if (cp->W > 0) s->read_set[(size_t)from * cp->W + (r >> 6)] |= 1ull << (r & 63);
    }
    POA_CTA_SYNC();

    POA_PAR_FOR(qi, qlen) {
        if ((kind_anchor[qi] >> 28) == CK_NEWM) {
            const int col = item_row[qi], id = tgt[qi];
            const int na = s->aln_cnt[col];
            if (na + 1 > A) POA_ATOMIC_OR(&s->failed, POA_CF_ALN_CAP);
            else {
                int32_t *mine = s->aln_id + (size_t)id * A; int nm = 0;
                for (int a = 0; a < na; ++a) {
                    const int sib = s->aln_id[(size_t)col * A + a];
                    s->aln_id[(size_t)sib * A + s->aln_cnt[sib]] = id; s->aln_cnt[sib] += 1;
                    mine[nm++] = sib;
                }
                s->aln_id[(size_t)col * A + na] = id; s->aln_cnt[col] = na + 1;
                mine[nm++] = col; s->aln_cnt[id] = nm;
            }
        }
    }
    POA_CTA_SYNC();
    if (s->failed) { if (POA_TID0) hdr->n_rows = 0; POA_CTA_SYNC(); return; }

    POA_PAR_FOR(k, n_new) { if (k > 0 && new_anchor[k] < new_anchor[k - 1]) POA_ATOMIC_OR(&s->failed, POA_CF_ORDER); }
    POA_CTA_SYNC();
// ... 260 lines not shown
```

### abpoa_b200/csrc/poa_kernels.cu

```cuda
#include <cuda_runtime.h>
#include <stdint.h>
#include <algorithm>
#include "poa_device.cuh"
#include "poa_chain.cuh"

#define FULL 0xffffffffu
#define NEG POA_NEG32

enum { LG = 0, AG = 1, CG = 2 };
enum { GLOBAL = 0, LOCAL = 1, EXTEND = 2 };

#define OP_M   0x1
#define OP_E1  0x2
#define OP_E2  0x4
#define OP_E   0x6
#define OP_F1  0x8
#define OP_F2  0x10
#define OP_F   0x18
#define OP_ALL 0x1f

__device__ __forceinline__ void ld8(const int16_t *p, int v[8]) {
    const uint4 u = *reinterpret_cast<const uint4 *>(p);
    v[0] = (int)(short)(u.x & 0xffff); v[1] = ((int)u.x) >> 16;
    v[2] = (int)(short)(u.y & 0xffff); v[3] = ((int)u.y) >> 16;
// ... 1363 lines not shown
                        cA = pg0 | (png << 12); cB = rowoff[prow].off; if (has_ps) c_ps = ldb(jv.predscore + pb + k);
                    }
                }
                const int nk = min(32, np - kb);
                for (int k = 0; k < nk; ++k) {
                    const unsigned A = __shfl_sync(FULL, cA, k), B = __shfl_sync(FULL, cB, k);
                    const int pg0 = (int)(A & 0xfffu), png = (int)((A >> 12) & 0x1fffu);
                    const bool near = (A >> 25) & 1u;
                    const int rel = g - pg0;
                    const bool inr = active && (unsigned)rel < (unsigned)png;
                    uint4 hp = make_uint4(NEGP2, NEGP2, NEGP2, NEGP2), ep1 = hp, ep2 = hp;
                    const uint32_t prs = ring_s + (A >> 26) * ring_row_bytes;
                    const ST *ph = planes + (size_t)B * POA_GROUP;
                    if (inr) {
                        if (near && rel < ring_groups) {
                            const uint32_t a = prs + (uint32_t)rel * 16u;
                            asm volatile("ld.shared.v4.u32 {%0,%1,%2,%3}, [%4];" : "=r"(hp.x), "=r"(hp.y), "=r"(hp.z), "=r"(hp.w) : "r"(a));
                            if (GAP != LG) asm volatile("ld.shared.v4.u32 {%0,%1,%2,%3}, [%4];" : "=r"(ep1.x), "=r"(ep1.y), "=r"(ep1.z), "=r"(ep1.w) : "r"(a + ring_plane_bytes));
                            if (GAP == CG) asm volatile("ld.shared.v4.u32 {%0,%1,%2,%3}, [%4];" : "=r"(ep2.x), "=r"(ep2.y), "=r"(ep2.z), "=r"(ep2.w) : "r"(a + 2 * ring_plane_bytes));
                        } else {
                            const ST *q = ph + (size_t)rel * POA_GROUP;
                            const size_t pp = (size_t)png * POA_GROUP;
                            hp = *reinterpret_cast<const uint4 *>(q);
                            if (GAP != LG) ep1 = *reinterpret_cast<const uint4 *>(q + (size_t)PL::E1 * pp);
                            if (GAP == CG) ep2 = *reinterpret_cast<const uint4 *>(q + (size_t)PL::E2 * pp);
                        }
                    }
                    unsigned prev = __shfl_up_sync(FULL, hp.w, 1);
                    if (lane == 0) {
                        int hm1 = NEGP;
                        if (fix_left) {
                            const int relm = rel - 1;
                            if ((unsigned)relm < (unsigned)png) {
                                if (near && relm < ring_groups) { unsigned short v; asm volatile("ld.shared.u16 %0, [%1];" : "=h"(v) : "r"(prs + (uint32_t)relm * 16u + 14u)); hm1 = (int)(short)v; }
                                else hm1 = (int)ph[(size_t)relm * POA_GROUP + 7];
                            }
                        }
                        if (MODE == LOCAL && g == 0) hm1 = 0;
                        prev = (unsigned)hm1 << 16;
                    }
                    unsigned d0 = sh1(prev, hp.x), d1 = sh1(hp.x, hp.y), d2 = sh1(hp.y, hp.z), d3 = sh1(hp.z, hp.w);
                    if (has_ps) {
                        const int ps = __shfl_sync(FULL, c_ps, k);
                        const unsigned ps2 = pk(ps, ps);
                        d0 = __viaddmax_s16x2(d0, ps2, NEGP2); d1 = __viaddmax_s16x2(d1, ps2, NEGP2);
                        d2 = __viaddmax_s16x2(d2, ps2, NEGP2); d3 = __viaddmax_s16x2(d3, ps2, NEGP2);
                        if (GAP == LG) {
                            hp.x = __viaddmax_s16x2(hp.x, ps2, NEGP2); hp.y = __viaddmax_s16x2(hp.y, ps2, NEGP2);
                            hp.z = __viaddmax_s16x2(hp.z, ps2, NEGP2); hp.w = __viaddmax_s16x2(hp.w, ps2, NEGP2);
                        } else {
                            ep1.x = __viaddmax_s16x2(ep1.x, ps2, NEGP2); ep1.y = __viaddmax_s16x2(ep1.y, ps2, NEGP2);
                            ep1.z = __viaddmax_s16x2(ep1.z, ps2, NEGP2); ep1.w = __viaddmax_s16x2(ep1.w, ps2, NEGP2);
                            if (GAP == CG) {
                                ep2.x = __viaddmax_s16x2(ep2.x, ps2, NEGP2); ep2.y = __viaddmax_s16x2(ep2.y, ps2, NEGP2);
                                ep2.z = __viaddmax_s16x2(ep2.z, ps2, NEGP2); ep2.w = __viaddmax_s16x2(ep2.w, ps2, NEGP2);
                            }
                        }
                    }
                    if (kb == 0 && k == 0) { D0[0] = d0; D0[1] = d1; D0[2] = d2; D0[3] = d3; }
                    M[0] = __vmaxs2(M[0], d0); M[1] = __vmaxs2(M[1], d1); M[2] = __vmaxs2(M[2], d2); M[3] = __vmaxs2(M[3], d3);
                    if (GAP == LG) {
                        X1[0] = __vmaxs2(X1[0], __viaddmax_s16x2(hp.x, kc.NE1, NEGP2)); X1[1] = __vmaxs2(X1[1], __viaddmax_s16x2(hp.y, kc.NE1, NEGP2));
                        X1[2] = __vmaxs2(X1[2], __viaddmax_s16x2(hp.z, kc.NE1, NEGP2)); X1[3] = __vmaxs2(X1[3], __viaddmax_s16x2(hp.w, kc.NE1, NEGP2));
                    } else {
                        X1[0] = __vmaxs2(X1[0], ep1.x); X1[1] = __vmaxs2(X1[1], ep1.y); X1[2] = __vmaxs2(X1[2], ep1.z); X1[3] = __vmaxs2(X1[3], ep1.w);
                        if (GAP == CG) { X2[0] = __vmaxs2(X2[0], ep2.x); X2[1] = __vmaxs2(X2[1], ep2.y); X2[2] = __vmaxs2(X2[2], ep2.z); X2[3] = __vmaxs2(X2[3], ep2.w); }
                    }
                }
            }

            KP(1)
            const int nlo = min(max(beg - g * 8, 0), 8), nhi = min(max(g * 8 + 7 - end, 0), 8);
            const uint4 clo = cap_lo[nlo], chi = cap_hi[nhi];
            const unsigned CLO[4] = { clo.x, clo.y, clo.z, clo.w };
            const unsigned CAP[4] = { __vmins2(clo.x, chi.x), __vmins2(clo.y, chi.y), __vmins2(clo.z, chi.z), __vmins2(clo.w, chi.w) };
            const unsigned S[4] = { sv.x, sv.y, sv.z, sv.w };

            unsigned H[4], F1[4], F2[4], E1o[4], E2o[4];
            p16_cells<GAP, MODE>(kc, CLO, CAP, S, M, X1, X2, (g - g0) * 8, e1, oe1, e2, oe2, zr2, lane, carry1, carry2, H, F1, F2, E1o, E2o);

            if (jd.btrec != nullptr) {
                unsigned t = 0;
#pragma unroll
                for (int k = 0; k < 4; ++k)
                    t |= __vcmpeq2(__viaddmax_s16x2(D0[k], S[k], NEGP2), H[k]) & (0x00020001u << (2 * k));
                const unsigned byte = (t | (t >> 16)) & 0xffu;
                uint8_t *rec = reinterpret_cast<uint8_t *>(jd.btrec + i);
                const int rel = g - g0;
                if (active && rel < POA_BTREC_GROUPS) rec[16 + rel] = (uint8_t)byte;
                if (lane == 0 && gp == g0)
                    *reinterpret_cast<uint4 *>(rec) = make_uint4((unsigned)(g0 * 8), (unsigned)mypred,
                                                                 (unsigned)rbase | (ngrp <= POA_BTREC_GROUPS ? 0x100u : 0u) | ((unsigned)min(ngrp, 0xffff) << 16), (unsigned)my_off);
            }
            KP(2)
            if (TMA && tma_row) {
                if (gp == g0) {
                    if (lane == 0) { if (ring_rows >= 8) asm volatile("cp.async.bulk.wait_group.read 7;" ::: "memory"); else asm volatile("cp.async.bulk.wait_group.read 0;" ::: "memory"); }
                    __syncwarp();
                }
                if (active) {
                    const uint32_t a = my_ring_s + (uint32_t)(g - g0) * 16u;
                    asm volatile("st.shared.v4.u32 [%0], {%1,%2,%3,%4};" :: "r"(a), "r"(H[0]), "r"(H[1]), "r"(H[2]), "r"(H[3]) : "memory");
                    if (GAP != LG) {
                        asm volatile("st.shared.v4.u32 [%0], {%1,%2,%3,%4};" :: "r"(a + (uint32_t)PL::E1 * ring_plane_bytes), "r"(E1o[0]), "r"(E1o[1]), "r"(E1o[2]), "r"(E1o[3]) : "memory");
                        asm volatile("st.shared.v4.u32 [%0], {%1,%2,%3,%4};" :: "r"(a + (uint32_t)PL::F1 * ring_plane_bytes), "r"(F1[0]), "r"(F1[1]), "r"(F1[2]), "r"(F1[3]) : "memory");
                    }
                    if (GAP == CG) {
                        asm volatile("st.shared.v4.u32 [%0], {%1,%2,%3,%4};" :: "r"(a + (uint32_t)PL::E2 * ring_plane_bytes), "r"(E2o[0]), "r"(E2o[1]), "r"(E2o[2]), "r"(E2o[3]) : "memory");
                        asm volatile("st.shared.v4.u32 [%0], {%1,%2,%3,%4};" :: "r"(a + (uint32_t)PL::F2 * ring_plane_bytes), "r"(F2[0]), "r"(F2[1]), "r"(F2[2]), "r"(F2[3]) : "memory");
                    }
                }
            } else
            if (active) {
                const int rel = g - g0;
                if (rel < ring_groups) {
                    const uint32_t a = my_ring_s + (uint32_t)rel * 16u;
                    asm volatile("st.shared.v4.u32 [%0], {%1,%2,%3,%4};" :: "r"(a), "r"(H[0]), "r"(H[1]), "r"(H[2]), "r"(H[3]) : "memory");
                    if (GAP != LG) asm volatile("st.shared.v4.u32 [%0], {%1,%2,%3,%4};" :: "r"(a + ring_plane_bytes), "r"(E1o[0]), "r"(E1o[1]), "r"(E1o[2]), "r"(E1o[3]) : "memory");
                    if (GAP == CG) asm volatile("st.shared.v4.u32 [%0], {%1,%2,%3,%4};" :: "r"(a + 2 * ring_plane_bytes), "r"(E2o[0]), "r"(E2o[1]), "r"(E2o[2]), "r"(E2o[3]) : "memory");
                }
                ST *q = rowp + (size_t)rel * POA_GROUP;
                *reinterpret_cast<uint4 *>(q) = make_uint4(H[0], H[1], H[2], H[3]);
                if (GAP != LG) *reinterpret_cast<uint4 *>(q + (size_t)PL::E1 * gplane) = make_uint4(E1o[0], E1o[1], E1o[2], E1o[3]);
                if (GAP == CG) *reinterpret_cast<uint4 *>(q + (size_t)PL::E2 * gplane) = make_uint4(E2o[0], E2o[1], E2o[2], E2o[3]);
                if (!FB && GAP != LG) *reinterpret_cast<uint4 *>(q + (size_t)PL::F1 * gplane) = make_uint4(F1[0], F1[1], F1[2], F1[3]);
                if (!FB && GAP == CG) *reinterpret_cast<uint4 *>(q + (size_t)PL::F2 * gplane) = make_uint4(F2[0], F2[1], F2[2], F2[3]);
            }

            KP(3)
            {
                const int lmax = active ? lane_max8(H) : NEGP;
                unsigned eq = 0;
#pragma unroll
                for (int k = 0; k < 4; ++k) { eq |= (unsigned)(lo16(H[k]) == lmax) << (2 * k); eq |= (unsigned)(hi16(H[k]) == lmax) << (2 * k + 1); }
                const int lfirst = g * 8 + __ffs(eq) - 1, llast = g * 8 + 31 - __clz(eq);
                const int pm = __reduce_max_sync(FULL, lmax);
                const unsigned bm = __ballot_sync(FULL, lmax == pm && pm > NEGP);
                if (bm) {
                    const int pl = __shfl_sync(FULL, lfirst, __ffs(bm) - 1);
                    const int pr = __shfl_sync(FULL, llast, 31 - __clz(bm));
                    if (pm > row_max) { row_max = pm; row_left = pl; row_right = pr; }
                    else if (pm == row_max) row_right = pr;
                }
            }
        }
        KP(4)
        if (TMA && tma_row) {
            asm volatile("fence.proxy.async.shared::cta;" ::: "memory");
            __syncwarp();
            if (lane == 0) {
                const uint32_t bytes = (uint32_t)ngrp * 16u;
#pragma unroll
                for (int pl = 0; pl < PL::N; ++pl)
                    asm volatile("cp.async.bulk.global.shared::cta.bulk_group [%0], [%1], %2;"
                                 :: "l"(rowp + (size_t)pl * gplane), "r"(my_ring_s + (uint32_t)pl * ring_plane_bytes), "r"(bytes) : "memory");
                asm volatile("cp.async.bulk.commit_group;" ::: "memory");
            }
        }
        if (lane == 0) {
            ring_meta[i & rmask] = make_uint4((unsigned)beg, (unsigned)end, (unsigned)(row_left + 1) | ((unsigned)(row_right + 1) << 16), my_off);
            PoaRowInfo ri; ri.beg = beg; ri.end = end; ri.left = row_left; ri.right = row_right;
            rowinfo[i] = ri; { PoaRowOff z; z.off = my_off; z.p0 = mypred; *reinterpret_cast<uint2 *>(rowoff + i) = make_uint2(z.off, (unsigned)z.p0); }
        }
        guard_lo |= (row_max < -14000); guard_hi |= (row_max > 29000);
        if (MODE == LOCAL) {
            if (row_max > best_score) { best_score = row_max; best_i = i; best_j = row_left; }
        } else if (MODE == EXTEND) {
            if (row_max > best_score) { best_score = row_max; best_i = i; best_j = row_right; best_row = i; }
            else if (prm->zdrop > 0) {
                const int delta = jv.remain(best_row) - rem;
                if (best_score - row_max > prm->zdrop + e1 * abs(delta - (row_right - best_j))) stop = true;
            }
        }
        __syncwarp();
        }
        asm volatile("" : "+r"(m2.x), "+r"(m2.y), "+r"(n_raw_pred), "+r"(n_raw_ps));
        pb = pe; pe = m2.x; rbase = n_rbase; rem = n_rem; nx_y = m2.y; raw_pred = n_raw_pred; raw_ps = n_raw_ps;
#pragma unroll
        for (int k = 0; k < LP; ++k) {
            lp_c[k] = LEAN ? __shfl_sync(FULL, lane < pe - pb ? raw_pred : -1, k) : -1;
            lps_c[k] = PS ? __shfl_sync(FULL, lane < pe - pb ? raw_ps : 0, k) : 0;
        }
    }
    cursor = cur32;
    KP_OUT(res)
    if (TMA) {
        if (lane == 0) asm volatile("cp.async.bulk.wait_group 0;" ::: "memory");
        __syncwarp();
    }

    if (MODE == GLOBAL) {
        const int sb = jv.predoff(n_rows - 1), sn = jv.predoff(n_rows) - sb;
        for (int k = 0; k < sn; ++k) {
            const int prow = jv.pred[sb + k];
            const PoaRowInfo pi = rowinfo[prow];
            const int endc = qlen > pi.end ? pi.end : qlen;
            const int pg0 = pi.beg >> 3;
            const int v = (endc >= pi.beg) ? (int)planes[(size_t)rowoff[prow].off * POA_GROUP + (endc - pg0 * 8)] : NEG;
            if (v > best_score) { best_score = v; best_i = prow; best_j = endc; }
        }
    }
    res.best_score = best_score; res.best_i = best_i; res.best_j = best_j;
    res.cells = cells; res.max_band = max_band; res.plane_units_used = cursor;
    if (guard_lo || guard_hi || best_score <= NEGP + 2000) res.status = POA_ST_RANGE;
    if (banded && MODE != LOCAL && (int64_t)max_band * max(e1, e2) + max(oe1, oe2) > 15000) res.status = POA_ST_RANGE;
    const long long clk1 = clock64();
    res.fwd_clk = clk1 - clk0;
#ifndef POA_KPROF
    { unsigned smid; asm volatile("mov.u32 %0, %%smid;" : "=r"(smid)); res.prof[5] = (int64_t)smid; }
#endif
    if (lane == 0) *jd.result = res;
    __syncwarp();
    if (prm->ret_cigar && res.status == POA_ST_OK) {
        FbCtx fx;
        fx.kc = &kc; fx.cap_lo = cap_lo; fx.cap_hi = cap_hi;
        fx.buf = reinterpret_cast<uint8_t *>(ring_data); fx.buf_cells = (int)ring_row_bytes * ring_rows;
        poa_backtrack<GAP, ST, MODE, FB, PS>(jv, jd, prm, mat_s, lane, best_i, best_j, *jd.result, 3, jd.btrec, &fx);
        if (lane == 0) jd.result->bt_clk = clock64() - clk1;
    }
}


#ifndef POA_P16_MINB
#define POA_P16_MINB 10
#endif
#define POA_P16_BOUNDS __launch_bounds__(32, POA_P16_MINB)
template <int GAP, int MODE, bool LEAN, bool TMA>
__global__ void POA_P16_BOUNDS poa_align_kernel_p16(const PoaJobDesc *__restrict__ jobs, const PoaParamsDev *__restrict__ prm,
                                                           int n_jobs, int ring_rows, int ring_cells, const __grid_constant__ P16Consts kc) {
    extern __shared__ __align__(16) uint8_t dyn_smem[];
    const int lane = threadIdx.x;
    const int job = blockIdx.x;
    if (job >= n_jobs) return;
    const P16Smem sm = p16_smem_init(dyn_smem, prm, ring_rows, lane);
    const PoaJobDesc jd = jobs[job];
    p16_run_job<GAP, MODE, LEAN, TMA>(jd, prm, kc, sm, ring_rows, ring_cells, lane);
    __syncwarp();
    if (lane == 0) signal_done(jd);
}

static inline size_t ring_smem_bytes(int gap, int bits, int ring_rows, int ring_cells, int all_planes = 0);

template <int GAP, bool STRAND, bool PS>
__device__ __forceinline__ void chain_align_read(const PoaJobDesc &jd, const PoaChainSlot *sl, const PoaChainParams *__restrict__ cp,
                                                 const PoaParamsDev *__restrict__ prm, const P16Consts &kc, const P16Smem &sm, int ring_rows, int ring_cells,
                                                 int lane) {
    PoaJobDesc jp = jd;
    bool second = false;
    for (int pass = 0; pass < (STRAND ? 2 : 1); ++pass) {
        p16_run_job<GAP, GLOBAL, true, false, true, PS>(jp, prm, kc, sm, ring_rows, ring_cells, lane);
        __syncwarp();
        if (!STRAND || pass) break;
        const PoaJobHeader *h = reinterpret_cast<const PoaJobHeader *>(jd.blob);
        const int qlen = h->qlen;
        if (jd.result->status != POA_ST_OK || !chain_weak_hit(jd.result->best_score, qlen, h->n_rows, cp->max_mat)) break;
        const uint8_t *q = sl->reads + sl->read_off[sl->fused];
        uint8_t *qs = const_cast<uint8_t *>(jd.blob) + h->off_qs;
        for (int k = lane; k < qlen; k += 32) qs[1 + k] = chain_comp(q[qlen - 1 - k]);
        __syncwarp();
        jp.cigar = sl->rc_cigar; jp.result = sl->rc_result;
        second = true;
    }
    if (!STRAND) return;
    int rc = 0;
    if (second) {
        const PoaResultDev *f = jd.result, *b = sl->rc_result;
        rc = b->status == POA_ST_OK && b->best_score > f->best_score;
        if (rc) for (int t = lane; t < b->n_ops; t += 32) jd.cigar[t] = sl->rc_cigar[t];
        __syncwarp();
        if (lane == 0) {
            PoaResultDev out = rc ? *b : *f;
            out.status = f->status != POA_ST_OK ? f->status : b->status;
            out.cells = f->cells + b->cells; out.fwd_clk = f->fwd_clk + b->fwd_clk; out.bt_clk = f->bt_clk + b->bt_clk;
            *jd.result = out;
        }
    }
    if (lane == 0) sl->read_rc[sl->fused] = (uint8_t)(rc | (second ? 2 : 0));
    __syncwarp();
}

template <int GAP, bool STRAND, bool PS>
__global__ void POA_P16_BOUNDS poa_chain_align_kernel_p16(const PoaChainSlot *__restrict__ slots, const int32_t *__restrict__ idx,
                                                           const PoaChainParams *__restrict__ cp, const PoaParamsDev *__restrict__ prm, int n_jobs,
                                                           int round, int ring_rows, int ring_cells, const __grid_constant__ P16Consts kc) {
    extern __shared__ __align__(16) uint8_t dyn_smem[];
    const int lane = threadIdx.x;
    const int job = blockIdx.x;
    if (job >= n_jobs) return;
    const PoaChainSlot *sl = &slots[idx[job]];
    if (job == 0 && lane == 0 && sl->pool_cursor) sl->pool_cursor[(round + 1) & 1] = 0ull;
    const PoaJobDesc jd = sl->jd;
    const int n_rows = reinterpret_cast<const PoaJobHeader *>(jd.blob)->n_rows;
    if (sl->failed || sl->fused >= sl->n_reads || n_rows < 3) { if (lane == 0) jd.result->status = POA_ST_SKIP; return; }
    const P16Smem sm = p16_smem_init(dyn_smem, prm, ring_rows, lane);
    chain_align_read<GAP, STRAND, PS>(jd, sl, cp, prm, kc, sm, ring_rows, ring_cells, lane);
}

__device__ __forceinline__ int chain_ld_relaxed(const int32_t *p) { int v; asm volatile("ld.relaxed.gpu.global.s32 %0, [%1];" : "=r"(v) : "l"(p) : "memory"); return v; }
__device__ __forceinline__ void chain_st_relaxed(int32_t *p, int v) { asm volatile("st.relaxed.gpu.global.s32 [%0], %1;" :: "l"(p), "r"(v) : "memory"); }
__device__ __forceinline__ unsigned long long chain_now_ns() { unsigned long long t; asm volatile("mov.u64 %0, %%globaltimer;" : "=l"(t)); return t; }

template <int GAP, bool STRAND, bool PS>
__global__ void POA_P16_BOUNDS poa_chain_dp_worker_kernel(PoaChainSlot *slots, PoaChainSync *sync, const PoaChainParams *__restrict__ cp,
                                                          const PoaParamsDev *__restrict__ prm, int n_groups, int ring_rows, int ring_cells, int dbg,
                                                          const __grid_constant__ P16Consts kc) {
    extern __shared__ __align__(16) uint8_t dyn_smem[];
    const int lane = threadIdx.x;
    const int g = blockIdx.x;
    if (g >= n_groups) return;
    PoaChainSlot *sl = &slots[g];
    const P16Smem sm = p16_smem_init(dyn_smem, prm, ring_rows, lane);
    const unsigned long long limit = sync->watchdog_ns;
    int pushed = 0;
    unsigned long long waited = 0;
    for (;;) {
        int state = 0;
        {
            const unsigned long long t0 = chain_now_ns();
            unsigned ns = 500, polls = 0;
            for (;;) {
                const int v = __shfl_sync(0xffffffffu, chain_ld_relaxed(&sl->turn), 0);
                if (v == 0) break;
                __nanosleep(ns); if (ns < 8000) ns <<= 1;
                if ((++polls & 63u) == 0) {
                    const int a = __shfl_sync(0xffffffffu, chain_ld_relaxed(&sync->abort), 0);
                    const unsigned late = __shfl_sync(0xffffffffu, (unsigned)(chain_now_ns() - t0 > limit), 0);
                    if (a) { state = 2; break; }
                    if (late) { if (lane == 0) chain_st_relaxed(&sync->abort, 1); state = 2; break; }
                }
            }
            waited += chain_now_ns() - t0;
        }
        if (state) break;
        if (!(dbg & 1)) __threadfence();
        const PoaJobDesc jd = sl->jd;
        const int n_rows = reinterpret_cast<const PoaJobHeader *>(jd.blob)->n_rows;
        if (sl->failed || sl->fused >= sl->n_reads || n_rows < 3) break;
        chain_align_read<GAP, STRAND, PS>(jd, sl, cp, prm, kc, sm, ring_rows, ring_cells, lane);
        __syncwarp();
        if (!(dbg & 1)) __threadfence();
        if (lane == 0) {
            chain_st_relaxed(&sl->turn, 1);
            const unsigned slot = atomicAdd(&sync->q_tail, 1u);
            chain_st_relaxed(&sync->tasks[slot], g);
        }
        ++pushed;
        __syncwarp();
    }
    if (lane == 0) {
        const int never = sl->n_reads - 1 - pushed;
        if (never > 0) atomicSub(&sync->total, never);
        sl->wait_ns = waited;
    }
}

template <int GAP, bool STRAND, bool PS>
static cudaError_t launch_chain_worker_one(PoaChainSlot *slots, PoaChainSync *sync, int n_groups, const PoaChainParams *cp, const PoaParamsDev *prm,
                                           int ring_rows, int ring_cells, const P16Consts &kc, cudaStream_t st) {
    static const int dbg = [] { const char *e = getenv("ABPOA_GPU_CHAIN_DBG"); return e && *e ? atoi(e) : 0; }();
    const size_t smem0 = ring_smem_bytes(GAP, 16, ring_rows, ring_cells) + 18 * sizeof(uint4);
    const size_t smem = (dbg & 2) ? smem0 : std::max<size_t>(smem0, (size_t)23 * 1024);
    cudaError_t e = cudaFuncSetAttribute(poa_chain_dp_worker_kernel<GAP, STRAND, PS>, cudaFuncAttributeMaxDynamicSharedMemorySize, (int)(227 * 1024));
    if (e != cudaSuccess) return e;
    { const char *cv = getenv("ABPOA_GPU_CHAIN_CARVEOUT");
      e = cudaFuncSetAttribute(poa_chain_dp_worker_kernel<GAP, STRAND, PS>, cudaFuncAttributePreferredSharedMemoryCarveout, cv && *cv ? atoi(cv) : (int)cudaSharedmemCarveoutMaxShared);
      if (e != cudaSuccess) return e; }
    poa_chain_dp_worker_kernel<GAP, STRAND, PS><<<n_groups, 32, smem, st>>>(slots, sync, cp, prm, n_groups, ring_rows, ring_cells, dbg, kc);
    return cudaGetLastError();
}
template <bool STRAND, bool PS>
static cudaError_t launch_chain_worker_gap(int gap_mode, PoaChainSlot *slots, PoaChainSync *sync, int n_groups, const PoaChainParams *cp,
                                           const PoaParamsDev *prm, int ring_rows, int ring_cells, const P16Consts &kc, cudaStream_t st) {
    if (gap_mode == LG) return launch_chain_worker_one<LG, STRAND, PS>(slots, sync, n_groups, cp, prm, ring_rows, ring_cells, kc, st);
    if (gap_mode == AG) return launch_chain_worker_one<AG, STRAND, PS>(slots, sync, n_groups, cp, prm, ring_rows, ring_cells, kc, st);
    return launch_chain_worker_one<CG, STRAND, PS>(slots, sync, n_groups, cp, prm, ring_rows, ring_cells, kc, st);
}
extern "C" cudaError_t poa_launch_chain_dp_worker(int gap_mode, const int *gaps, PoaChainSlot *slots, PoaChainSync *sync, int n_groups,
                                                  const PoaChainParams *cp, int strand, int ps, const PoaParamsDev *prm, int ring_rows, int ring_cells,
                                                  cudaStream_t st) {
    if (n_groups <= 0) return cudaSuccess;
    const P16Consts kc = make_p16_consts(gaps[0], gaps[1], gaps[2], gaps[3]);
    if (strand) return ps ? launch_chain_worker_gap<true, true>(gap_mode, slots, sync, n_groups, cp, prm, ring_rows, ring_cells, kc, st)
                          : launch_chain_worker_gap<true, false>(gap_mode, slots, sync, n_groups, cp, prm, ring_rows, ring_cells, kc, st);
    return ps ? launch_chain_worker_gap<false, true>(gap_mode, slots, sync, n_groups, cp, prm, ring_rows, ring_cells, kc, st)
              : launch_chain_worker_gap<false, false>(gap_mode, slots, sync, n_groups, cp, prm, ring_rows, ring_cells, kc, st);
}

template <int GAP, bool STRAND, bool PS>
static cudaError_t launch_chain_one(const PoaChainSlot *slots, const int32_t *idx, int n_jobs, int round, const PoaChainParams *cp, const PoaParamsDev *prm,
                                    int ring_rows, int ring_cells, const P16Consts &kc, cudaStream_t st) {
    const size_t smem = ring_smem_bytes(GAP, 16, ring_rows, ring_cells) + 18 * sizeof(uint4);
    cudaError_t e = cudaFuncSetAttribute(poa_chain_align_kernel_p16<GAP, STRAND, PS>, cudaFuncAttributeMaxDynamicSharedMemorySize, (int)(227 * 1024));
    if (e != cudaSuccess) return e;
    poa_chain_align_kernel_p16<GAP, STRAND, PS><<<n_jobs, 32, smem, st>>>(slots, idx, cp, prm, n_jobs, round, ring_rows, ring_cells, kc);
    return cudaGetLastError();
}
template <bool STRAND, bool PS>
static cudaError_t launch_chain_gap(int gap_mode, const PoaChainSlot *slots, const int32_t *idx, int n_jobs, int round, const PoaChainParams *cp,
                                    const PoaParamsDev *prm, int ring_rows, int ring_cells, const P16Consts &kc, cudaStream_t st) {
    if (gap_mode == LG) return launch_chain_one<LG, STRAND, PS>(slots, idx, n_jobs, round, cp, prm, ring_rows, ring_cells, kc, st);
    if (gap_mode == AG) return launch_chain_one<AG, STRAND, PS>(slots, idx, n_jobs, round, cp, prm, ring_rows, ring_cells, kc, st);
    return launch_chain_one<CG, STRAND, PS>(slots, idx, n_jobs, round, cp, prm, ring_rows, ring_cells, kc, st);
}
extern "C" cudaError_t poa_launch_chain_align_p16(int gap_mode, const int *gaps, const PoaChainSlot *slots, const int32_t *idx, int n_jobs, int round,
                                                  const PoaChainParams *cp, int strand, int ps, const PoaParamsDev *prm, int ring_rows, int ring_cells,
                                                  cudaStream_t st) {
    if (n_jobs <= 0) return cudaSuccess;
    const P16Consts kc = make_p16_consts(gaps[0], gaps[1], gaps[2], gaps[3]);
    if (strand) return ps ? launch_chain_gap<true, true>(gap_mode, slots, idx, n_jobs, round, cp, prm, ring_rows, ring_cells, kc, st)
                          : launch_chain_gap<true, false>(gap_mode, slots, idx, n_jobs, round, cp, prm, ring_rows, ring_cells, kc, st);
    return ps ? launch_chain_gap<false, true>(gap_mode, slots, idx, n_jobs, round, cp, prm, ring_rows, ring_cells, kc, st)
              : launch_chain_gap<false, false>(gap_mode, slots, idx, n_jobs, round, cp, prm, ring_rows, ring_cells, kc, st);
}

template <int GAP, bool PS>
__global__ void POA_P16_BOUNDS poa_chain_replay_kernel(const __grid_constant__ PoaJobDesc jd, const PoaParamsDev *__restrict__ prm,
                                                       int ring_rows, int ring_cells, const __grid_constant__ P16Consts kc) {
    extern __shared__ __align__(16) uint8_t dyn_smem[];
    const int lane = threadIdx.x;
    const P16Smem sm = p16_smem_init(dyn_smem, prm, ring_rows, lane);
    p16_run_job<GAP, GLOBAL, true, false, true, PS>(jd, prm, kc, sm, ring_rows, ring_cells, lane);
}

template <int GAP, bool PS>
__global__ void __launch_bounds__(32) poa_fb_dump_kernel(const __grid_constant__ PoaJobDesc jd, const PoaParamsDev *__restrict__ prm, int buf_cells,
                                                         int16_t *fslab, uint8_t *fbits, int32_t *windows, const __grid_constant__ P16Consts kc) {
    extern __shared__ __align__(16) uint8_t dyn_smem[];
    const int lane = threadIdx.x, i = blockIdx.x + 1;
    const JobView jv = open_job(jd.blob);
    if (i >= jv.n_rows - 1) return;
    const P16Smem sm = p16_smem_init(dyn_smem, prm, 0, lane);
    const PoaRowInfo ri = jd.rowinfo[i];
    int n = 0;
    if (ri.end >= ri.beg) {
        const uint32_t off = jd.rowoff[i].off;
        const int g0 = ri.beg >> 3, ngrp = (ri.end >> 3) - g0 + 1;
        FbDumpCtx fx;
        fx.kc = &kc; fx.cap_lo = sm.cap_lo; fx.cap_hi = sm.cap_hi;
        fx.buf = reinterpret_cast<uint8_t *>(sm.ring_data); fx.buf_cells = buf_cells;
        fx.f = fslab + (size_t)off * POA_GROUP; fx.fstride = ngrp * POA_GROUP;
        const int2 m0 = ldb(jv.rowmeta + i);
        const int np = ldb(&jv.rowmeta[i + 1].x) - m0.x;
        uint8_t *ob = fbits + (size_t)off * POA_GROUP;
        for (int j = ri.end; j >= ri.beg; ++n) {
            const int lo = fb_recompute<GAP, GLOBAL, true, PS>(jv, jd, prm, fx, ri.beg, ri.end, m0.x, np, m0.y & 0xff, j, lane);
            for (int c = lo + lane; c <= j; c += 32) ob[c - g0 * 8] = fx.buf[c - lo];
            __syncwarp();
            j = lo - 1;
        }
    }
    if (lane == 0) windows[i] = n;
}

#define POA_SMEM_MAX (227 * 1024)
template <int GAP, bool PS>
static cudaError_t launch_chain_replay_one(const PoaJobDesc &jd, const PoaParamsDev *prm, int ring_rows, int ring_cells, const P16Consts &kc, cudaStream_t st) {
    const size_t smem = ring_smem_bytes(GAP, 16, ring_rows, ring_cells) + 18 * sizeof(uint4);
    if (smem > POA_SMEM_MAX) return cudaErrorInvalidValue;
    cudaError_t e = cudaFuncSetAttribute(poa_chain_replay_kernel<GAP, PS>, cudaFuncAttributeMaxDynamicSharedMemorySize, POA_SMEM_MAX);
    if (e != cudaSuccess) return e;
    poa_chain_replay_kernel<GAP, PS><<<1, 32, smem, st>>>(jd, prm, ring_rows, ring_cells, kc);
    return cudaGetLastError();
}
extern "C" cudaError_t poa_launch_chain_replay(int gap_mode, const int *gaps, const PoaJobDesc *jd, const PoaParamsDev *prm, int ring_rows, int ring_cells,
                                               int ps, cudaStream_t st) {
    if (gap_mode == LG || ring_rows < 2 || (ring_rows & (ring_rows - 1)) || ring_cells < 8 || (ring_cells & 7)) return cudaErrorInvalidValue;
    const P16Consts kc = make_p16_consts(gaps[0], gaps[1], gaps[2], gaps[3]);
    if (gap_mode == AG) return ps ? launch_chain_replay_one<AG, true>(*jd, prm, ring_rows, ring_cells, kc, st) : launch_chain_replay_one<AG, false>(*jd, prm, ring_rows, ring_cells, kc, st);
    return ps ? launch_chain_replay_one<CG, true>(*jd, prm, ring_rows, ring_cells, kc, st) : launch_chain_replay_one<CG, false>(*jd, prm, ring_rows, ring_cells, kc, st);
}
extern "C" int poa_chain_fb_buf_cells(int gap_mode, int ring_rows, int ring_cells) {
    const int rn = gap_mode == LG ? RingPlanes<LG>::N : (gap_mode == AG ? RingPlanes<AG>::N : RingPlanes<CG>::N);
    return rn * ring_cells * 2 * ring_rows;
}
template <int GAP, bool PS>
static cudaError_t launch_fb_dump_one(const PoaJobDesc &jd, const PoaParamsDev *prm, int n_rows, int buf_cells, int16_t *fslab, uint8_t *fbits,
                                      int32_t *windows, const P16Consts &kc, cudaStream_t st) {
    const size_t smem = (size_t)POA_MAX_M * POA_MAX_M * sizeof(int) + 18 * sizeof(uint4) + (size_t)std::max(buf_cells >> 8, 1) * 256;
    if (smem > POA_SMEM_MAX) return cudaErrorInvalidValue;
    cudaError_t e = cudaFuncSetAttribute(poa_fb_dump_kernel<GAP, PS>, cudaFuncAttributeMaxDynamicSharedMemorySize, POA_SMEM_MAX);
    if (e != cudaSuccess) return e;
    if (n_rows > 2) poa_fb_dump_kernel<GAP, PS><<<n_rows - 2, 32, smem, st>>>(jd, prm, buf_cells, fslab, fbits, windows, kc);
    return cudaGetLastError();
}
extern "C" cudaError_t poa_launch_fb_dump(int gap_mode, const int *gaps, const PoaJobDesc *jd, const PoaParamsDev *prm, int n_rows, int buf_cells,
                                          int16_t *fslab, uint8_t *fbits, int32_t *windows, int ps, cudaStream_t st) {
    if (gap_mode == LG) return cudaErrorInvalidValue;
    const P16Consts kc = make_p16_consts(gaps[0], gaps[1], gaps[2], gaps[3]);
    if (gap_mode == AG) return ps ? launch_fb_dump_one<AG, true>(*jd, prm, n_rows, buf_cells, fslab, fbits, windows, kc, st)
                                  : launch_fb_dump_one<AG, false>(*jd, prm, n_rows, buf_cells, fslab, fbits, windows, kc, st);
    return ps ? launch_fb_dump_one<CG, true>(*jd, prm, n_rows, buf_cells, fslab, fbits, windows, kc, st)
              : launch_fb_dump_one<CG, false>(*jd, prm, n_rows, buf_cells, fslab, fbits, windows, kc, st);
}

static inline size_t ring_smem_bytes(int gap, int bits, int ring_rows, int ring_cells, int all_planes) {
    const int rn = all_planes ? (gap == LG ? 1 : (gap == AG ? 3 : 5)) : (gap == LG ? 1 : (gap == AG ? 2 : 3));
    return (size_t)POA_MAX_M * POA_MAX_M * sizeof(int) + (size_t)ring_rows * sizeof(PoaRowInfo) + (((size_t)ring_rows * 4 + 15) & ~(size_t)15)
           + (size_t)ring_rows * rn * ring_cells * (bits / 8);
}

template <int GAP, typename ST, int MODE>
static cudaError_t launch_one(const PoaJobDesc *jobs, const PoaParamsDev *prm, int n_jobs, int ring_rows, int ring_cells, cudaStream_t st) {
    const size_t smem = ring_smem_bytes(GAP, (int)sizeof(ST) * 8, ring_rows, ring_cells);
    cudaError_t e = cudaFuncSetAttribute(poa_align_kernel<GAP, ST, MODE>, cudaFuncAttributeMaxDynamicSharedMemorySize, (int)(227 * 1024));
    if (e != cudaSuccess) return e;
    const char *cv = getenv("ABPOA_GPU_CARVEOUT");
    if (cv && *cv) cudaFuncSetAttribute(poa_align_kernel<GAP, ST, MODE>, cudaFuncAttributePreferredSharedMemoryCarveout, atoi(cv));
    poa_align_kernel<GAP, ST, MODE><<<n_jobs, 32, smem, st>>>(jobs, prm, n_jobs, ring_rows, ring_cells);
    return cudaGetLastError();
}

template <int GAP, typename ST>
static cudaError_t launch_mode(int mode, const PoaJobDesc *jobs, const PoaParamsDev *prm, int n_jobs, int rr, int rc, cudaStream_t st) {
    switch (mode) {
    case GLOBAL: return launch_one<GAP, ST, GLOBAL>(jobs, prm, n_jobs, rr, rc, st);
    case LOCAL:  return launch_one<GAP, ST, LOCAL>(jobs, prm, n_jobs, rr, rc, st);
    default:     return launch_one<GAP, ST, EXTEND>(jobs, prm, n_jobs, rr, rc, st);
    }
}

extern "C" int poa_tma_enabled(void) { static const int on = [] { const char *e = getenv("ABPOA_GPU_TMA"); return e && *e == '1'; }(); return on; }
extern "C" int poa_lean_disabled(void) { static const int off = [] { const char *e = getenv("ABPOA_GPU_NO_LEAN"); return e && *e == '1'; }(); return off; }
extern "C" void poa_pick_ring(int gap_mode, int bits, int band_cells, size_t smem_budget, int *ring_rows, int *ring_cells) {
    int rc = band_cells < 64 ? 64 : band_cells;
    int rr = 64;
    const int all = bits == 16 && poa_tma_enabled();
    if (all) smem_budget += 12 * 1024;
    smem_budget = smem_budget > 512 ? smem_budget - 512 : smem_budget;
    while (rr > 2 && ring_smem_bytes(gap_mode, bits, rr, rc, all) > smem_budget) rr >>= 1;
    while (rc > 64 && ring_smem_bytes(gap_mode, bits, rr, rc, all) > smem_budget) rc -= 64;
    *ring_rows = rr; *ring_cells = rc;
}

template <int GAP, int MODE, bool LEAN, bool TMA>
static cudaError_t launch_p16_one(const PoaJobDesc *jobs, const PoaParamsDev *prm, int n_jobs, int ring_rows, int ring_cells, const P16Consts &kc, cudaStream_t st) {
    const size_t smem = ring_smem_bytes(GAP, 16, ring_rows, ring_cells, TMA) + 18 * sizeof(uint4);
    cudaError_t e = cudaFuncSetAttribute(poa_align_kernel_p16<GAP, MODE, LEAN, TMA>, cudaFuncAttributeMaxDynamicSharedMemorySize, (int)(227 * 1024));
    if (e != cudaSuccess) return e;
    const char *cv = getenv("ABPOA_GPU_CARVEOUT");
    if (cv && *cv) cudaFuncSetAttribute(poa_align_kernel_p16<GAP, MODE, LEAN, TMA>, cudaFuncAttributePreferredSharedMemoryCarveout, atoi(cv));
    poa_align_kernel_p16<GAP, MODE, LEAN, TMA><<<n_jobs, 32, smem, st>>>(jobs, prm, n_jobs, ring_rows, ring_cells, kc);
    return cudaGetLastError();
}
template <int GAP>
static cudaError_t launch_p16_mode(int mode, int lean, const PoaJobDesc *jobs, const PoaParamsDev *prm, int n_jobs, int rr, int rc, const P16Consts &kc, cudaStream_t st) {
    switch (mode) {
    case GLOBAL:
        if (lean && poa_tma_enabled()) return launch_p16_one<GAP, GLOBAL, true, true>(jobs, prm, n_jobs, rr, rc, kc, st);
        return lean ? launch_p16_one<GAP, GLOBAL, true, false>(jobs, prm, n_jobs, rr, rc, kc, st) : launch_p16_one<GAP, GLOBAL, false, false>(jobs, prm, n_jobs, rr, rc, kc, st);
    case LOCAL:  return launch_p16_one<GAP, LOCAL, false, false>(jobs, prm, n_jobs, rr, rc, kc, st);
    default:     return launch_p16_one<GAP, EXTEND, false, false>(jobs, prm, n_jobs, rr, rc, kc, st);
    }
}
extern "C" cudaError_t poa_launch_align_p16(int gap_mode, int align_mode, int lean, const int *gaps, const PoaJobDesc *jobs,
                                            const PoaParamsDev *prm, int n_jobs, int ring_rows, int ring_cells, cudaStream_t st) {
    if (n_jobs <= 0) return cudaSuccess;
    const P16Consts kc = make_p16_consts(gaps[0], gaps[1], gaps[2], gaps[3]);
    if (poa_lean_disabled()) lean = 0;
    if (gap_mode == LG) return launch_p16_mode<LG>(align_mode, lean, jobs, prm, n_jobs, ring_rows, ring_cells, kc, st);
    if (gap_mode == AG) return launch_p16_mode<AG>(align_mode, lean, jobs, prm, n_jobs, ring_rows, ring_cells, kc, st);
    return launch_p16_mode<CG>(align_mode, lean, jobs, prm, n_jobs, ring_rows, ring_cells, kc, st);
}

extern "C" cudaError_t poa_launch_align(int gap_mode, int bits, int align_mode, const PoaJobDesc *jobs,
                                        const PoaParamsDev *prm, int n_jobs, int ring_rows, int ring_cells, cudaStream_t st) {
    if (n_jobs <= 0) return cudaSuccess;
    if (bits == 16) {
        if (gap_mode == LG) return launch_mode<LG, int16_t>(align_mode, jobs, prm, n_jobs, ring_rows, ring_cells, st);
        if (gap_mode == AG) return launch_mode<AG, int16_t>(align_mode, jobs, prm, n_jobs, ring_rows, ring_cells, st);
        return launch_mode<CG, int16_t>(align_mode, jobs, prm, n_jobs, ring_rows, ring_cells, st);
    }
    if (gap_mode == LG) return launch_mode<LG, int32_t>(align_mode, jobs, prm, n_jobs, ring_rows, ring_cells, st);
    if (gap_mode == AG) return launch_mode<AG, int32_t>(align_mode, jobs, prm, n_jobs, ring_rows, ring_cells, st);
    return launch_mode<CG, int32_t>(align_mode, jobs, prm, n_jobs, ring_rows, ring_cells, st);
}
```

Baseline: 126.6.

## Replace per-group DP warps with persistent workers pulling from a ready queue

The alignment worker kernel no longer launches one warp per group that spins on its own turn flag. It now launches a persistent grid sized by occupancy. Workers pull ready group ids from a global queue that the seed and fuse kernels push to, and the number of active workers per SM is limited so the fuse kernel still fits. This targets idle warps spinning and load imbalance between groups. The CTA scans and the remain-row tile also now process four items per thread, and an optional per-worker stats log was added. The cost is more atomics on the shared queue and a more complex handoff protocol between the two kernels.

```diff
diff --git a/abpoa_b200/csrc/poa_chain.cu b/abpoa_b200/csrc/poa_chain.cu
--- a/abpoa_b200/csrc/poa_chain.cu
+++ b/abpoa_b200/csrc/poa_chain.cu
@@ -20,22 +20,25 @@
 #define CK(call) do { cudaError_t e_ = (call); if (e_ != cudaSuccess) \
     poa_die("libabpoa_b200/chain", "%s failed at %s:%d: %s", #call, __FILE__, __LINE__, cudaGetErrorString(e_)); } while (0)
 
-extern "C" cudaError_t poa_launch_chain_dp_worker(int gap_mode, const int *gaps, PoaChainSlot *slots, PoaChainSync *sync, int n_groups,
+extern "C" cudaError_t poa_launch_chain_dp_worker(int gap_mode, const int *gaps, PoaChainSlot *slots, PoaChainSync *sync, int n_groups, int sm_count,
+                                                  const int *fuse_res,
                                                   const PoaChainParams *cp, int strand, int ps, const PoaParamsDev *prm, int ring_rows, int ring_cells,
-                                                  cudaStream_t st);
+                                                  cudaStream_t st, int *n_workers);
 extern "C" cudaError_t poa_launch_chain_align_p16(int gap_mode, const int *gaps, const PoaChainSlot *slots, const int32_t *idx, int n_jobs, int round,
                                                   const PoaChainParams *cp, int strand, int ps, const PoaParamsDev *prm, int ring_rows, int ring_cells,
                                                   cudaStream_t st);
 extern "C" void poa_pick_ring(int gap_mode, int bits, int band_cells, size_t smem_budget, int *ring_rows, int *ring_cells);
 
-static_assert(offsetof(PoaChainSync, q_tail) == 128 && offsetof(PoaChainSync, total) == 256 && offsetof(PoaChainSync, abort) == 384,
+static_assert(offsetof(PoaChainSync, q_tail) == 128 && offsetof(PoaChainSync, total) == 256 && offsetof(PoaChainSync, abort) == 384 &&
+              offsetof(PoaChainSync, r_head) == 512 && offsetof(PoaChainSync, r_tail) == 640 && offsetof(PoaChainSync, r_total) == 768,
               "every polled / bumped word of PoaChainSync sits in its own 128-byte line");
 static_assert(POA_GFA_HDR_WORDS == POA_GFA_HDR, "the device's GFA record header is the one poa_gfa_from_record reads");
 
 template <bool PS>
-__global__ void __launch_bounds__(POA_CHAIN_T) poa_chain_seed_kernel(PoaChainSlot *slots, const PoaChainParams *cp, int n) {
+__global__ void __launch_bounds__(POA_CHAIN_T) poa_chain_seed_kernel(PoaChainSlot *slots, const PoaChainParams *cp, int n, PoaChainSync *sync) {
     if ((int)blockIdx.x >= n) return;
     chain_seed<PS>(&slots[blockIdx.x], cp);
+    if (sync && threadIdx.x == 0) chain_hand_on(&slots[blockIdx.x], sync, (int)blockIdx.x);
 }
 
 template <bool PS>
@@ -83,7 +86,7 @@
         __syncthreads();
         __threadfence();
         __syncthreads();
-        if (threadIdx.x == 0) { s->fuse_ns += sync_now_ns() - t0; __threadfence(); sync_st(&s->turn, 0); }
+        if (threadIdx.x == 0) { s->fuse_ns += sync_now_ns() - t0; chain_hand_on(s, sync, g); }
     }
 }
 
@@ -410,7 +413,8 @@
     uint8_t *d_base = NULL; size_t total = 0, doff = 0;
     PoaChainSlot *d_slots = NULL; PoaChainParams *d_cp = NULL; PoaParamsDev *d_prm = NULL;
     unsigned long long *d_cursors = NULL;
-    PoaChainSync *d_sync = NULL; int32_t *d_tasks = NULL; int64_t n_tasks = 0;
+    PoaChainSync *d_sync = NULL; int32_t *d_tasks = NULL, *d_ready = NULL, *d_sm_workers = NULL; int64_t n_tasks = 0;
+    PoaChainWorkerStat *d_wstat = NULL; int n_workers = 0;
     uint8_t *d_reads = NULL; size_t reads_bytes = 0;
     int32_t *d_idx = NULL; size_t idx_n = 0;
     int64_t *d_exoff = NULL, *d_msaoff = NULL, *d_gfaoff = NULL; int32_t *d_excap = NULL;
@@ -472,6 +476,9 @@
         d_sync = (PoaChainSync *)dtake(sizeof(PoaChainSync));
         for (int t = 0; t < nw; ++t) n_tasks += plans[t].n_reads - 1;
         d_tasks = (int32_t *)dtake((size_t)std::max<int64_t>(n_tasks, 1) * 4);
+        d_ready = (int32_t *)dtake((size_t)std::max<int64_t>(n_tasks, 1) * 4);
+        d_sm_workers = (int32_t *)dtake((size_t)POA_CHAIN_MAX_SMID * 4);
+        d_wstat = (PoaChainWorkerStat *)dtake((size_t)POA_CHAIN_MAX_WORKERS_PER_SM * c.sm_count * sizeof(PoaChainWorkerStat));
         for (int t = 0; t < nw; ++t) reads_bytes += plans[t].reads_bytes;
         h_reads = (uint8_t *)pinned_get(0, reads_bytes + 256);
         d_reads = dtake(reads_bytes);
@@ -539,7 +546,7 @@
         return true;
     }
 
-    void upload_and_seed(const std::vector<int32_t> &idx) {
+    void upload_and_seed(const std::vector<int32_t> &idx, const PoaChainSync *hsync = NULL) {
         for (Cohort &k : coh) { CK(cudaStreamCreateWithFlags(&k.st, cudaStreamNonBlocking)); CK(cudaEventCreate(&k.ev_end)); }
         s0 = coh[0].st;
         CK(cudaEventCreateWithFlags(&ev_up, cudaEventDisableTiming)); CK(cudaEventCreate(&ev_t0)); CK(cudaEventCreate(&ev_t1));
@@ -557,10 +564,18 @@
         CK(cudaMemcpyAsync(d_exoff, h_exoff.data(), (size_t)nw * 8, cudaMemcpyHostToDevice, s0));
         CK(cudaMemcpyAsync(d_excap, h_excap.data(), (size_t)nw * 4, cudaMemcpyHostToDevice, s0));
         CK(cudaMemsetAsync(d_cursors, 0, (size_t)32 * sizeof(unsigned long long), s0));
+        if (hsync) {
+            const size_t qb = (size_t)std::max<int64_t>(n_tasks, 1) * 4;
+            CK(cudaMemcpyAsync(d_sync, hsync, sizeof *hsync, cudaMemcpyHostToDevice, s0));
+            CK(cudaMemsetAsync(d_tasks, 0xff, qb, s0)); CK(cudaMemsetAsync(d_ready, 0xff, qb, s0));
+            CK(cudaMemsetAsync(d_sm_workers, 0, (size_t)POA_CHAIN_MAX_SMID * 4, s0));
+            CK(cudaMemsetAsync(d_wstat, 0xff, (size_t)POA_CHAIN_MAX_WORKERS_PER_SM * c.sm_count * sizeof(PoaChainWorkerStat), s0));
+        }
         h2d = reads_bytes + (uint64_t)nw * sizeof(PoaChainSlot) + sizeof hcp + sizeof hprm + idx.size() * 4 + (uint64_t)nw * 12;
         CK(cudaEventRecord(ev_t0, s0));
-        if (c.ps) poa_chain_seed_kernel<true><<<nw, POA_CHAIN_T, 0, s0>>>(d_slots, d_cp, nw);
-        else poa_chain_seed_kernel<false><<<nw, POA_CHAIN_T, 0, s0>>>(d_slots, d_cp, nw);
+        PoaChainSync *seed_sync = hsync ? d_sync : NULL;
+        if (c.ps) poa_chain_seed_kernel<true><<<nw, POA_CHAIN_T, 0, s0>>>(d_slots, d_cp, nw, seed_sync);
+        else poa_chain_seed_kernel<false><<<nw, POA_CHAIN_T, 0, s0>>>(d_slots, d_cp, nw, seed_sync);
         CK(cudaGetLastError());
         CK(cudaEventRecord(ev_up, s0));
         static const size_t smem_budget = [] { const char *e = getenv("ABPOA_GPU_SMEM_KB"); return (size_t)(e && *e ? atoi(e) : 28) * 1024; }();
@@ -583,13 +598,12 @@
             hs[t].pool_base = d_pool + o; hs[t].pool_units = share / 16; hs[t].pool_cursor = NULL;
             o += share;
         }
-        upload_and_seed({});
         static const double watchdog_s = [] { const char *e = getenv("ABPOA_GPU_CHAIN_WATCHDOG_S"); return e && *e ? atof(e) : 30.0; }();
+        PoaChainSync hsync; memset(&hsync, 0, sizeof hsync);
+        hsync.total = hsync.r_total = (int32_t)n_tasks; hsync.watchdog_ns = (unsigned long long)(watchdog_s * 1e9);
+        hsync.tasks = d_tasks; hsync.ready = d_ready; hsync.sm_workers = d_sm_workers; hsync.wstat = d_wstat;
+        upload_and_seed({}, &hsync);
         static const int fuse_per_sm = [] { const char *e = getenv("ABPOA_GPU_CHAIN_FUSE_PER_SM"); return e && *e ? std::max(1, atoi(e)) : 1; }();
-        PoaChainSync hsync; memset(&hsync, 0, sizeof hsync);
-        hsync.total = (int32_t)n_tasks; hsync.watchdog_ns = (unsigned long long)(watchdog_s * 1e9); hsync.tasks = d_tasks;
-        CK(cudaMemcpyAsync(d_sync, &hsync, sizeof hsync, cudaMemcpyHostToDevice, s0));
-        CK(cudaMemsetAsync(d_tasks, 0xff, (size_t)std::max<int64_t>(n_tasks, 1) * 4, s0));
         CK(cudaStreamCreateWithFlags(&st_dp, cudaStreamNonBlocking));
         cudaEvent_t ev_sync; CK(cudaEventCreateWithFlags(&ev_sync, cudaEventDisableTiming));
         CK(cudaEventRecord(ev_sync, s0));
@@ -597,13 +611,15 @@
         const int n_fuse = std::max(1, std::min(std::min(nw, c.sm_count * fuse_per_sm), fuse_cap));
         CK(cudaFuncSetAttribute(c.ps ? poa_chain_fuse_worker_kernel<true> : poa_chain_fuse_worker_kernel<false>, cudaFuncAttributePreferredSharedMemoryCarveout,
                                 cudaSharedmemCarveoutMaxShared));
+        cudaFuncAttributes fa; CK(cudaFuncGetAttributes(&fa, c.ps ? poa_chain_fuse_worker_kernel<true> : poa_chain_fuse_worker_kernel<false>));
+        const int fuse_res[2] = { fa.numRegs, (int)fa.sharedSizeBytes };
         static const bool dp_first = [] { const char *e = getenv("ABPOA_GPU_CHAIN_DP_FIRST"); return e && *e == '1'; }();
         CK(cudaStreamWaitEvent(st_dp, ev_sync, 0));
-        if (dp_first) CK(poa_launch_chain_dp_worker(c.abpt->gap_mode, gaps, d_slots, d_sync, nw, d_cp, c.strand, c.ps, d_prm, ring_rows, ring_cells, st_dp));
+        if (dp_first) CK(poa_launch_chain_dp_worker(c.abpt->gap_mode, gaps, d_slots, d_sync, nw, c.sm_count, fuse_res, d_cp, c.strand, c.ps, d_prm, ring_rows, ring_cells, st_dp, &n_workers));
         if (c.ps) poa_chain_fuse_worker_kernel<true><<<n_fuse, POA_CHAIN_T, 0, s0>>>(d_slots, d_sync, d_cp);
         else poa_chain_fuse_worker_kernel<false><<<n_fuse, POA_CHAIN_T, 0, s0>>>(d_slots, d_sync, d_cp);
         CK(cudaGetLastError());
-        if (!dp_first) CK(poa_launch_chain_dp_worker(c.abpt->gap_mode, gaps, d_slots, d_sync, nw, d_cp, c.strand, c.ps, d_prm, ring_rows, ring_cells, st_dp));
+        if (!dp_first) CK(poa_launch_chain_dp_worker(c.abpt->gap_mode, gaps, d_slots, d_sync, nw, c.sm_count, fuse_res, d_cp, c.strand, c.ps, d_prm, ring_rows, ring_cells, st_dp, &n_workers));
         cudaEvent_t ev_dp; CK(cudaEventCreateWithFlags(&ev_dp, cudaEventDisableTiming));
         CK(cudaEventRecord(ev_dp, st_dp));
         CK(cudaStreamWaitEvent(s0, ev_dp, 0));
@@ -692,6 +708,7 @@
             PoaChainSync hs2; CK(cudaMemcpy(&hs2, d_sync, sizeof hs2, cudaMemcpyDeviceToHost));
             if (hs2.abort) fprintf(stderr, "[libabpoa_b200/chain] watchdog: the alignment and the fuse kernel did not make progress together within ABPOA_GPU_CHAIN_WATCHDOG_S; "
                                            "unfinished groups go to the launch engine (ABPOA_GPU_CHAIN_ROUNDS=1 selects the round schedule)\n");
+            sched_log();
         }
         t_dev_done = now_ms();
         recoff.assign((size_t)nw, -1); msaoff.assign((size_t)nw, -1); gfaoff.assign((size_t)nw, -1);
@@ -748,6 +765,28 @@
         d2h = (uint64_t)tot_words * 4 + (uint64_t)cons_words * 4 + (uint64_t)nw * (sizeof(PoaChainSlot) + 16) + rc_bytes;
         poa_arena_return(c.arena, d_base, total); d_base = NULL;
         t_copied = now_ms();
+    }
+
+    void sched_log() {
+        static const char *path = getenv("ABPOA_GPU_CHAIN_SCHED_LOG");
+        if (!path || !*path || n_workers <= 0) return;
+        std::vector<PoaChainWorkerStat> ws((size_t)n_workers);
+        CK(cudaMemcpy(ws.data(), d_wstat, ws.size() * sizeof(PoaChainWorkerStat), cudaMemcpyDeviceToHost));
+        static std::mutex mu;
+        std::lock_guard<std::mutex> lk(mu);
+        FILE *f = fopen(path, "a");
+        if (!f) return;
+        fprintf(f, "{\"groups\": %d, \"sm_count\": %d, \"grid\": %d, \"workers\": [", nw, c.sm_count, n_workers);
+        bool first = true;
+        for (const PoaChainWorkerStat &w : ws) {
+            if (w.smid < 0) continue;
+            fprintf(f, "%s[%d, %d, %llu, %llu, %llu]", first ? "" : ", ", w.smid, w.n_jobs, w.t_first_ns, w.t_last_ns, w.busy_ns);
+            first = false;
+        }
+        fprintf(f, "], \"group_done_ns\": [");
+        for (int t = 0; t < nw; ++t) fprintf(f, "%s%llu", t ? ", " : "", fin[t].t_task_ns);
+        fprintf(f, "]}\n");
+        fclose(f);
     }
 
     void install() {
diff --git a/abpoa_b200/csrc/poa_chain.cuh b/abpoa_b200/csrc/poa_chain.cuh
--- a/abpoa_b200/csrc/poa_chain.cuh
+++ b/abpoa_b200/csrc/poa_chain.cuh
@@ -66,8 +66,9 @@
     const int32_t *read_w;
     PoaJobDesc jd;
     uint8_t *pool_base; unsigned long long *pool_cursor; uint64_t pool_units;
-    int32_t turn;
+    int32_t jobs;
     int32_t rsv0;
+    unsigned long long t_task_ns;
     unsigned long long wait_ns, fuse_ns;
     int64_t prof[6];
     int64_t btdiag[5];
@@ -116,14 +117,43 @@
     if (qv) s->read_qw = (const uint8_t *)take((size_t)bases);
 }
 
+typedef struct PoaChainWorkerStat {
+    int32_t smid, n_jobs;
+    unsigned long long t_first_ns, t_last_ns;
+    unsigned long long busy_ns;
+} PoaChainWorkerStat;
+
+#define POA_CHAIN_MAX_SMID 1024
+#define POA_CHAIN_MAX_WORKERS_PER_SM 32
+
 typedef struct PoaChainSync {
     unsigned int q_head; int32_t pad0[31];
     unsigned int q_tail; int32_t pad1[31];
     int32_t total; int32_t pad2[31];
     int32_t abort; int32_t pad3[31];
+    unsigned int r_head; int32_t pad4[31];
+    unsigned int r_tail; int32_t pad5[31];
+    int32_t r_total; int32_t pad6[31];
     unsigned long long watchdog_ns;
-    int32_t *tasks;
+    int32_t *tasks, *ready;
+    int32_t *sm_workers;
+    PoaChainWorkerStat *wstat;
 } PoaChainSync;
+
+#ifndef POA_CHAIN_EMUL
+__device__ inline void chain_hand_on(PoaChainSlot *s, PoaChainSync *sync, int g) {
+    const int n_rows = reinterpret_cast<const PoaJobHeader *>(s->jd.blob)->n_rows;
+    if (!s->failed && s->fused < s->n_reads && n_rows >= 3) {
+        s->jobs += 1;
+        __threadfence();
+        const unsigned at = atomicAdd(&sync->r_tail, 1u);
+        asm volatile("st.relaxed.gpu.global.s32 [%0], %1;" :: "l"(sync->ready + at), "r"(g) : "memory");
+    } else {
+        const int never = s->n_reads - 1 - s->jobs;
+        if (never > 0) { atomicSub(&sync->total, never); atomicSub(&sync->r_total, never); }
+    }
+}
+#endif
 
 #ifdef POA_CHAIN_EMUL
 POA_DEV int cta_excl_scan(int32_t *a, int n) {
@@ -136,15 +166,18 @@
     for (int i = 0; i < n; ++i) { if (a[i] > run) run = a[i]; a[i] = run; }
 }
 #else
+#define POA_SCAN_ITEMS 4
 __device__ inline int cta_excl_scan(int32_t *a, int n) {
     __shared__ int warp_sum[32];
     __shared__ int carry_s;
     const int lane = threadIdx.x & 31, wid = threadIdx.x >> 5, nw = blockDim.x >> 5;
     if (threadIdx.x == 0) carry_s = 0;
     __syncthreads();
-    for (int base = 0; base < n; base += blockDim.x) {
-        const int i = base + threadIdx.x;
-        const int v = i < n ? a[i] : 0;
+    for (int base = 0; base < n; base += POA_SCAN_ITEMS * blockDim.x) {
+        const int i0 = base + POA_SCAN_ITEMS * threadIdx.x;
+        int e[POA_SCAN_ITEMS], v = 0;
+#pragma unroll
+        for (int k = 0; k < POA_SCAN_ITEMS; ++k) { e[k] = i0 + k < n ? a[i0 + k] : 0; v += e[k]; }
         int x = v;
 #pragma unroll
         for (int d = 1; d < 32; d <<= 1) { const int t = __shfl_up_sync(0xffffffffu, x, d); if (lane >= d) x += t; }
@@ -158,8 +191,9 @@
         }
         __syncthreads();
         const int carry = carry_s;
-        const int before = carry + (wid > 0 ? warp_sum[wid - 1] : 0) + x - v;
-        if (i < n) a[i] = before;
+        int before = carry + (wid > 0 ? warp_sum[wid - 1] : 0) + x - v;
+#pragma unroll
+        for (int k = 0; k < POA_SCAN_ITEMS; ++k) { if (i0 + k < n) a[i0 + k] = before; before += e[k]; }
         __syncthreads();
         if (threadIdx.x == 0) carry_s = carry + warp_sum[nw - 1];
         __syncthreads();
@@ -172,9 +206,11 @@
     const int lane = threadIdx.x & 31, wid = threadIdx.x >> 5, nw = blockDim.x >> 5;
     if (threadIdx.x == 0) carry_m = INT32_MIN;
     __syncthreads();
-    for (int base = 0; base < n; base += blockDim.x) {
-        const int i = base + threadIdx.x;
-        int x = i < n ? a[i] : INT32_MIN;
+    for (int base = 0; base < n; base += POA_SCAN_ITEMS * blockDim.x) {
+        const int i0 = base + POA_SCAN_ITEMS * threadIdx.x;
+        int e[POA_SCAN_ITEMS], x = INT32_MIN;
+#pragma unroll
+        for (int k = 0; k < POA_SCAN_ITEMS; ++k) { e[k] = i0 + k < n ? a[i0 + k] : INT32_MIN; x = max(x, e[k]); }
 #pragma unroll
         for (int d = 1; d < 32; d <<= 1) { const int t = __shfl_up_sync(0xffffffffu, x, d); if (lane >= d) x = max(x, t); }
         if (lane == 31) warp_max[wid] = x;
@@ -186,9 +222,11 @@
             warp_max[lane] = s;
         }
         __syncthreads();
-        int r = max(carry_m, x);
+        int ex = __shfl_up_sync(0xffffffffu, x, 1);
+        int r = lane > 0 ? max(carry_m, ex) : carry_m;
         if (wid > 0) r = max(r, warp_max[wid - 1]);
-        if (i < n) a[i] = r;
+#pragma unroll
+        for (int k = 0; k < POA_SCAN_ITEMS; ++k) { r = max(r, e[k]); if (i0 + k < n) a[i0 + k] = r; }
         __syncthreads();
         if (threadIdx.x == 0) carry_m = max(carry_m, warp_max[nw - 1]);
         __syncthreads();
@@ -252,15 +290,16 @@
 
 POA_DEV int chain_read_weight(const ChainRead &rd, int qi) { return !rd.w ? 1 : rd.w[rd.rc ? rd.len - 1 - qi : qi]; }
 
+#define POA_REMAIN_TILE (4 * POA_CHAIN_T)
 POA_DEV void chain_set_remain(PoaChainSlot *s, int K, const int32_t *order, int n) {
-    POA_SHARED int t_ptr[POA_CHAIN_T], t_val[POA_CHAIN_T], t_np[POA_CHAIN_T], t_nv[POA_CHAIN_T];
+    POA_SHARED int t_ptr[POA_REMAIN_TILE], t_val[POA_REMAIN_TILE], t_np[POA_REMAIN_TILE], t_nv[POA_REMAIN_TILE];
     int32_t *rem = s->rem_row;
     if (POA_TID0) rem[n - 1] = -1;
     POA_CTA_SYNC();
-    for (int hi = n - 1; hi > 0; hi -= POA_CHAIN_T) {
-        const int lo = hi - POA_CHAIN_T > 0 ? hi - POA_CHAIN_T : 0;
+    for (int hi = n - 1; hi > 0; hi -= POA_REMAIN_TILE) {
+        const int lo = hi - POA_REMAIN_TILE > 0 ? hi - POA_REMAIN_TILE : 0;
         const int cnt = hi - lo;
-        POA_PAR_FOR(l, POA_CHAIN_T) {
+        POA_PAR_FOR(l, POA_REMAIN_TILE) {
             if (l < cnt) {
                 const int v = order[lo + l];
                 const int sr = s->node_row[s->out_id[(size_t)v * K]];
@@ -269,16 +308,16 @@
             } else { t_ptr[l] = -1; t_val[l] = 0; }
         }
         POA_CTA_SYNC();
-        for (int step = 1; step < POA_CHAIN_T; step <<= 1) {
-            POA_PAR_FOR(l, POA_CHAIN_T) {
+        for (int step = 1; step < POA_REMAIN_TILE; step <<= 1) {
+            POA_PAR_FOR(l, POA_REMAIN_TILE) {
                 const int p = t_ptr[l];
                 if (p >= 0) { t_nv[l] = t_val[l] + t_val[p]; t_np[l] = t_ptr[p]; } else { t_nv[l] = t_val[l]; t_np[l] = -1; }
             }
             POA_CTA_SYNC();
-            POA_PAR_FOR(l, POA_CHAIN_T) { t_val[l] = t_nv[l]; t_ptr[l] = t_np[l]; }
+            POA_PAR_FOR(l, POA_REMAIN_TILE) { t_val[l] = t_nv[l]; t_ptr[l] = t_np[l]; }
             POA_CTA_SYNC();
         }
-        POA_PAR_FOR(l, POA_CHAIN_T) { if (l < cnt) rem[lo + l] = t_val[l]; }
+        POA_PAR_FOR(l, POA_REMAIN_TILE) { if (l < cnt) rem[lo + l] = t_val[l]; }
         POA_CTA_SYNC();
     }
 }
diff --git a/abpoa_b200/csrc/poa_kernels.cu b/abpoa_b200/csrc/poa_kernels.cu
--- a/abpoa_b200/csrc/poa_kernels.cu
+++ b/abpoa_b200/csrc/poa_kernels.cu
@@ -1689,88 +1689,120 @@
 
 template <int GAP, bool STRAND, bool PS>
 __global__ void POA_P16_BOUNDS poa_chain_dp_worker_kernel(PoaChainSlot *slots, PoaChainSync *sync, const PoaChainParams *__restrict__ cp,
-                                                          const PoaParamsDev *__restrict__ prm, int n_groups, int ring_rows, int ring_cells, int dbg,
+                                                          const PoaParamsDev *__restrict__ prm, int per_sm, int ring_rows, int ring_cells, int dbg,
                                                           const __grid_constant__ P16Consts kc) {
     extern __shared__ __align__(16) uint8_t dyn_smem[];
     const int lane = threadIdx.x;
-    const int g = blockIdx.x;
-    if (g >= n_groups) return;
-    PoaChainSlot *sl = &slots[g];
+    unsigned smid; asm volatile("mov.u32 %0, %%smid;" : "=r"(smid));
+    int stay = 0;
+    if (lane == 0) stay = smid >= POA_CHAIN_MAX_SMID || atomicAdd(&sync->sm_workers[smid], 1) < per_sm;
+    if (!__shfl_sync(0xffffffffu, stay, 0)) return;
     const P16Smem sm = p16_smem_init(dyn_smem, prm, ring_rows, lane);
     const unsigned long long limit = sync->watchdog_ns;
-    int pushed = 0;
-    unsigned long long waited = 0;
+    if (lane == 0) {
+        PoaChainWorkerStat *ws = sync->wstat + blockIdx.x;
+        ws->smid = (int32_t)smid; ws->n_jobs = 0; ws->t_first_ns = ws->t_last_ns = ws->busy_ns = 0;
+    }
     for (;;) {
-        int state = 0;
+        unsigned ticket = 0;
+        if (lane == 0) ticket = atomicAdd(&sync->r_head, 1u);
+        ticket = __shfl_sync(0xffffffffu, ticket, 0);
+        int g = -1;
         {
-            const unsigned long long t0 = chain_now_ns();
-            unsigned ns = 500, polls = 0;
+            unsigned long long t0 = chain_now_ns();
+            unsigned ns = 500, polls = 0, seen = 0;
             for (;;) {
-                const int v = __shfl_sync(0xffffffffu, chain_ld_relaxed(&sl->turn), 0);
-                if (v == 0) break;
+                if ((polls++ & 63u) == 0) {
+                    const int tot = __shfl_sync(0xffffffffu, chain_ld_relaxed(&sync->r_total), 0), a = __shfl_sync(0xffffffffu, chain_ld_relaxed(&sync->abort), 0);
+                    if ((long long)ticket >= (long long)tot || a) break;
+                    const unsigned tail = __shfl_sync(0xffffffffu, (unsigned)chain_ld_relaxed(reinterpret_cast<const int32_t *>(&sync->r_tail)), 0);
+                    const unsigned long long now = __shfl_sync(0xffffffffu, chain_now_ns(), 0);
+                    if (polls == 1 || tail != seen) { seen = tail; t0 = now; }
+                    else if (now - t0 > limit) { if (lane == 0) chain_st_relaxed(&sync->abort, 1); break; }
+                }
+                g = __shfl_sync(0xffffffffu, chain_ld_relaxed(&sync->ready[ticket]), 0);
+                if (g >= 0) break;
                 __nanosleep(ns); if (ns < 8000) ns <<= 1;
-                if ((++polls & 63u) == 0) {
-                    const int a = __shfl_sync(0xffffffffu, chain_ld_relaxed(&sync->abort), 0);
-                    const unsigned late = __shfl_sync(0xffffffffu, (unsigned)(chain_now_ns() - t0 > limit), 0);
-                    if (a) { state = 2; break; }
-                    if (late) { if (lane == 0) chain_st_relaxed(&sync->abort, 1); state = 2; break; }
-                }
-            }
-            waited += chain_now_ns() - t0;
-        }
-        if (state) break;
+            }
+        }
+        if (g < 0) break;
         if (!(dbg & 1)) __threadfence();
+        PoaChainSlot *sl = &slots[g];
+        const unsigned long long t_pick = chain_now_ns();
+        if (lane == 0 && sl->jobs > 1) sl->wait_ns += t_pick - sl->t_task_ns;
         const PoaJobDesc jd = sl->jd;
-        const int n_rows = reinterpret_cast<const PoaJobHeader *>(jd.blob)->n_rows;
-        if (sl->failed || sl->fused >= sl->n_reads || n_rows < 3) break;
         chain_align_read<GAP, STRAND, PS>(jd, sl, cp, prm, kc, sm, ring_rows, ring_cells, lane);
         __syncwarp();
+        const unsigned long long t_done = chain_now_ns();
+        if (lane == 0) sl->t_task_ns = t_done;
         if (!(dbg & 1)) __threadfence();
         if (lane == 0) {
-            chain_st_relaxed(&sl->turn, 1);
             const unsigned slot = atomicAdd(&sync->q_tail, 1u);
             chain_st_relaxed(&sync->tasks[slot], g);
         }
-        ++pushed;
+        if (lane == 0) {
+            PoaChainWorkerStat *ws = sync->wstat + blockIdx.x;
+            if (!ws->n_jobs) ws->t_first_ns = t_pick;
+            ws->n_jobs += 1; ws->t_last_ns = t_done; ws->busy_ns += t_done - t_pick;
+        }
         __syncwarp();
     }
-    if (lane == 0) {
-        const int never = sl->n_reads - 1 - pushed;
-        if (never > 0) atomicSub(&sync->total, never);
-        sl->wait_ns = waited;
-    }
+}
+
+static int chain_workers_per_sm(int n_groups, int sm_count, int resident, int k_regs, size_t k_smem, int fuse_regs, size_t fuse_smem) {
+    int dev = 0, smem_sm = 0, rsv = 0, regs_sm = 0;
+    if (cudaGetDevice(&dev) != cudaSuccess || cudaDeviceGetAttribute(&smem_sm, cudaDevAttrMaxSharedMemoryPerMultiprocessor, dev) != cudaSuccess ||
+        cudaDeviceGetAttribute(&rsv, cudaDevAttrReservedSharedMemoryPerBlock, dev) != cudaSuccess ||
+        cudaDeviceGetAttribute(&regs_sm, cudaDevAttrMaxRegistersPerMultiprocessor, dev) != cudaSuccess)
+        return 1;
+    auto warp_regs = [](int r) { return (r * 32 + 255) / 256 * 256; };
+    const long smem_left = (long)smem_sm - (long)(fuse_smem + rsv), regs_left = (long)regs_sm - (long)warp_regs(fuse_regs) * (POA_CHAIN_T / 32);
+    const long fit = std::min<long>(resident, std::min(smem_left / (long)(k_smem + rsv), regs_left / warp_regs(k_regs)));
+    const long want = ((long)n_groups + sm_count - 1) / sm_count;
+    return (int)std::max(1L, std::min(fit, want));
 }
 
 template <int GAP, bool STRAND, bool PS>
-static cudaError_t launch_chain_worker_one(PoaChainSlot *slots, PoaChainSync *sync, int n_groups, const PoaChainParams *cp, const PoaParamsDev *prm,
-                                           int ring_rows, int ring_cells, const P16Consts &kc, cudaStream_t st) {
+static cudaError_t launch_chain_worker_one(PoaChainSlot *slots, PoaChainSync *sync, int n_groups, int sm_count, const int *fuse_res,
+                                           const PoaChainParams *cp, const PoaParamsDev *prm, int ring_rows, int ring_cells, const P16Consts &kc,
+                                           cudaStream_t st, int *n_workers) {
     static const int dbg = [] { const char *e = getenv("ABPOA_GPU_CHAIN_DBG"); return e && *e ? atoi(e) : 0; }();
     const size_t smem0 = ring_smem_bytes(GAP, 16, ring_rows, ring_cells) + 18 * sizeof(uint4);
     const size_t smem = (dbg & 2) ? smem0 : std::max<size_t>(smem0, (size_t)23 * 1024);
-    cudaError_t e = cudaFuncSetAttribute(poa_chain_dp_worker_kernel<GAP, STRAND, PS>, cudaFuncAttributeMaxDynamicSharedMemorySize, (int)(227 * 1024));
+    auto kern = poa_chain_dp_worker_kernel<GAP, STRAND, PS>;
+    cudaError_t e = cudaFuncSetAttribute(kern, cudaFuncAttributeMaxDynamicSharedMemorySize, (int)(227 * 1024));
     if (e != cudaSuccess) return e;
     { const char *cv = getenv("ABPOA_GPU_CHAIN_CARVEOUT");
-      e = cudaFuncSetAttribute(poa_chain_dp_worker_kernel<GAP, STRAND, PS>, cudaFuncAttributePreferredSharedMemoryCarveout, cv && *cv ? atoi(cv) : (int)cudaSharedmemCarveoutMaxShared);
+      e = cudaFuncSetAttribute(kern, cudaFuncAttributePreferredSharedMemoryCarveout, cv && *cv ? atoi(cv) : (int)cudaSharedmemCarveoutMaxShared);
       if (e != cudaSuccess) return e; }
-    poa_chain_dp_worker_kernel<GAP, STRAND, PS><<<n_groups, 32, smem, st>>>(slots, sync, cp, prm, n_groups, ring_rows, ring_cells, dbg, kc);
+    int resident = 0;
+    if ((e = cudaOccupancyMaxActiveBlocksPerMultiprocessor(&resident, kern, 32, smem)) != cudaSuccess) return e;
+    if (resident < 1) return cudaErrorInvalidConfiguration;
+    cudaFuncAttributes fa;
+    if ((e = cudaFuncGetAttributes(&fa, kern)) != cudaSuccess) return e;
+    const int per_sm = chain_workers_per_sm(n_groups, sm_count, resident, fa.numRegs, smem + fa.sharedSizeBytes, fuse_res[0], (size_t)fuse_res[1]);
+    *n_workers = resident * sm_count;
+    kern<<<resident * sm_count, 32, smem, st>>>(slots, sync, cp, prm, per_sm, ring_rows, ring_cells, dbg, kc);
     return cudaGetLastError();
 }
 template <bool STRAND, bool PS>
-static cudaError_t launch_chain_worker_gap(int gap_mode, PoaChainSlot *slots, PoaChainSync *sync, int n_groups, const PoaChainParams *cp,
-                                           const PoaParamsDev *prm, int ring_rows, int ring_cells, const P16Consts &kc, cudaStream_t st) {
-    if (gap_mode == LG) return launch_chain_worker_one<LG, STRAND, PS>(slots, sync, n_groups, cp, prm, ring_rows, ring_cells, kc, st);
-    if (gap_mode == AG) return launch_chain_worker_one<AG, STRAND, PS>(slots, sync, n_groups, cp, prm, ring_rows, ring_cells, kc, st);
-    return launch_chain_worker_one<CG, STRAND, PS>(slots, sync, n_groups, cp, prm, ring_rows, ring_cells, kc, st);
-}
-extern "C" cudaError_t poa_launch_chain_dp_worker(int gap_mode, const int *gaps, PoaChainSlot *slots, PoaChainSync *sync, int n_groups,
+static cudaError_t launch_chain_worker_gap(int gap_mode, PoaChainSlot *slots, PoaChainSync *sync, int n_groups, int sm_count, const int *fuse_res, const PoaChainParams *cp,
+                                           const PoaParamsDev *prm, int ring_rows, int ring_cells, const P16Consts &kc, cudaStream_t st, int *n_workers) {
+    if (gap_mode == LG) return launch_chain_worker_one<LG, STRAND, PS>(slots, sync, n_groups, sm_count, fuse_res, cp, prm, ring_rows, ring_cells, kc, st, n_workers);
+    if (gap_mode == AG) return launch_chain_worker_one<AG, STRAND, PS>(slots, sync, n_groups, sm_count, fuse_res, cp, prm, ring_rows, ring_cells, kc, st, n_workers);
+    return launch_chain_worker_one<CG, STRAND, PS>(slots, sync, n_groups, sm_count, fuse_res, cp, prm, ring_rows, ring_cells, kc, st, n_workers);
+}
+extern "C" cudaError_t poa_launch_chain_dp_worker(int gap_mode, const int *gaps, PoaChainSlot *slots, PoaChainSync *sync, int n_groups, int sm_count,
+                                                  const int *fuse_res,
                                                   const PoaChainParams *cp, int strand, int ps, const PoaParamsDev *prm, int ring_rows, int ring_cells,
-                                                  cudaStream_t st) {
+                                                  cudaStream_t st, int *n_workers) {
+    *n_workers = 0;
     if (n_groups <= 0) return cudaSuccess;
     const P16Consts kc = make_p16_consts(gaps[0], gaps[1], gaps[2], gaps[3]);
-    if (strand) return ps ? launch_chain_worker_gap<true, true>(gap_mode, slots, sync, n_groups, cp, prm, ring_rows, ring_cells, kc, st)
-                          : launch_chain_worker_gap<true, false>(gap_mode, slots, sync, n_groups, cp, prm, ring_rows, ring_cells, kc, st);
-    return ps ? launch_chain_worker_gap<false, true>(gap_mode, slots, sync, n_groups, cp, prm, ring_rows, ring_cells, kc, st)
-              : launch_chain_worker_gap<false, false>(gap_mode, slots, sync, n_groups, cp, prm, ring_rows, ring_cells, kc, st);
+    if (strand) return ps ? launch_chain_worker_gap<true, true>(gap_mode, slots, sync, n_groups, sm_count, fuse_res, cp, prm, ring_rows, ring_cells, kc, st, n_workers)
+                          : launch_chain_worker_gap<true, false>(gap_mode, slots, sync, n_groups, sm_count, fuse_res, cp, prm, ring_rows, ring_cells, kc, st, n_workers);
+    return ps ? launch_chain_worker_gap<false, true>(gap_mode, slots, sync, n_groups, sm_count, fuse_res, cp, prm, ring_rows, ring_cells, kc, st, n_workers)
+              : launch_chain_worker_gap<false, false>(gap_mode, slots, sync, n_groups, sm_count, fuse_res, cp, prm, ring_rows, ring_cells, kc, st, n_workers);
 }
 
 template <int GAP, bool STRAND, bool PS>
```

After: 129.3, median of 6. 1.02x the previous value.
